# nirvanesque/headCT_foundation

Measured on AMD Instinct MI355X. Metric: CT-volumes/sec MAE pretrain step (96^3, ViT-B/16^3, mask 0.75), higher is better.
Workload: dtype bf16; 1 GPU; BASELINE config #2: MAE ViT-B/16^3, 96^3x1ch, mask 0.75, full train step (fwd+bwd+clip+AdamW+LR); per_gpu_batch=256, global_batch=256, parallelism=dp1, init=reference init, seed 42

## Files before the change

### headct_foundation_amd/_lib.py

```python
from __future__ import annotations

import ctypes as C
import os
from typing import Optional

HERE = os.path.dirname(os.path.abspath(__file__))
LIB_PATH = os.path.join(HERE, "libheadct_hip.so")

HCT_F32, HCT_BF16, HCT_F16 = 0, 1, 2
NORM_LAYERNORM, NORM_RMSNORM = 0, 1
HCT_ACT_NONE, HCT_ACT_GELU, HCT_ACT_DGELU, HCT_ACT_TANH, HCT_ACT_GELU_D, HCT_ACT_MULAUX = 0, 1, 2, 3, 4, 5
ACT_NONE, ACT_GELU, ACT_DGELU = 0, 1, 2

c_void_p, c_int, c_float, c_size_t, c_int64 = C.c_void_p, C.c_int, C.c_float, C.c_size_t, C.c_int64


class GemmArgs(C.Structure):
    _fields_ = [
        ("M", c_int), ("N", c_int), ("K", c_int),
        ("A", c_void_p), ("a_dtype", c_int), ("lda", c_int64), ("transA", c_int),
        ("B", c_void_p), ("b_dtype", c_int), ("ldb", c_int64), ("transB", c_int),
        ("C", c_void_p), ("c_dtype", c_int), ("ldc", c_int64),
        ("bias", c_void_p), ("residual", c_void_p), ("ldr", c_int64),
        ("act", c_int),
# ... 58 lines not shown
    "hct_rmsnorm_fwd": (c_int, [c_void_p, c_void_p, c_int, c_int, c_float, c_void_p, c_int, c_void_p, c_void_p]),
    "hct_rmsnorm_bwd_workspace_bytes": (c_size_t, [c_int, c_int]),
    "hct_rmsnorm_bwd": (c_int, [c_void_p, c_int, c_void_p, c_void_p, c_void_p, c_void_p, c_int, c_int, c_void_p, c_void_p, c_int, c_void_p,
                                c_void_p, c_void_p, c_size_t, c_void_p]),
    "hct_rmsnorm_bwd_mapped": (c_int, [c_void_p, c_int, c_void_p, c_void_p, c_void_p, c_void_p, c_void_p, c_int, c_int, c_void_p, c_void_p,
                                       c_int, c_void_p, c_void_p, c_void_p, c_size_t, c_void_p]),
    "hct_tail_rows": (c_int, [c_void_p, c_int, c_int, c_int, c_void_p, c_void_p, c_void_p]),
    "hct_gather_rows": (c_int, [c_void_p, c_void_p, c_int, c_int, c_void_p, c_void_p]),
    "hct_attention_fwd": (c_int, [c_void_p, c_int, c_int, c_int, c_int, c_int, c_void_p, c_void_p, c_void_p]),
    "hct_attention_bwd": (c_int, [c_void_p, c_void_p, c_void_p, c_void_p, c_int, c_int, c_int, c_int, c_int, c_void_p, c_void_p]),
    "hct_debug_force_simple_attention": (None, [c_int]),
    "hct_decoder_assemble_fwd": (c_int, [c_void_p, c_int, c_void_p, c_void_p, c_void_p, c_void_p, c_int, c_int, c_int, c_int, c_void_p, c_void_p]),
    "hct_decoder_assemble_bwd": (c_int, [c_void_p, c_void_p, c_void_p, c_int, c_int, c_int, c_int, c_void_p, c_int, c_void_p, c_void_p,
                                         c_void_p, c_size_t, c_void_p]),
    "hct_masked_mse": (c_int, [c_void_p, c_int, c_void_p, c_int, c_void_p, c_int, c_int, c_int, c_int, c_int, c_float, c_void_p, c_void_p, c_void_p, c_void_p, c_void_p]),
    "hct_unpatchify": (c_int, [c_void_p, c_int, c_int, c_int, c_int, c_int, c_int, c_void_p, c_void_p]),
    "hct_vit_assemble_fwd": (c_int, [c_void_p, c_int, c_void_p, c_void_p, c_void_p, c_int, c_int, c_int, c_int, c_void_p, c_void_p]),
    "hct_channel_norm": (c_int, [c_void_p, c_void_p, c_void_p, c_float, c_void_p, c_int, c_int64, c_int, c_void_p]),
    "hct_query_attention": (c_int, [c_void_p, c_int, c_void_p, c_int, c_int, c_int, c_int, c_int, c_float, c_void_p, c_void_p]),
    "hct_head_linear": (c_int, [c_void_p, c_int64, c_int, c_void_p, c_void_p, c_float, c_void_p, c_void_p, c_int, c_void_p, c_int, c_int,
                                c_int, c_void_p]),
    "hct_batchnorm_stats": (c_int, [c_void_p, c_int, c_int, c_float, c_void_p, c_void_p, c_void_p, c_void_p, c_void_p]),
    "hct_softmax_xent": (c_int, [c_void_p, c_void_p, c_int, c_int, c_void_p, c_void_p, c_void_p, c_void_p]),
    "hct_head_linear_wgrad": (c_int, [c_void_p, c_void_p, c_void_p, c_float, c_void_p, c_int, c_int, c_int, c_void_p, c_void_p, c_void_p]),
    "hct_bn_rows_workspace_bytes": (c_size_t, [c_int, c_int]),
    "hct_bn_stats_rows": (c_int, [c_void_p, c_int, c_int64, c_int, c_int, c_float, c_void_p, c_void_p, c_void_p, c_void_p, c_void_p,
                                  c_size_t, c_void_p]),
    "hct_bn_norm": (c_int, [c_void_p, c_int, c_int64, c_int64, c_int, c_void_p, c_void_p, c_float, c_void_p, c_int, c_void_p]),
    "hct_bn_bwd_input": (c_int, [c_void_p, c_int, c_int64, c_void_p, c_void_p, c_float, c_void_p, c_int64, c_void_p, c_void_p, c_int,
                                 c_int, c_int, c_int, c_void_p, c_int, c_int64, c_void_p, c_size_t, c_void_p]),
    "hct_head_linear_x": (c_int, [c_void_p, c_int, c_int64, c_int, c_void_p, c_void_p, c_float, c_void_p, c_void_p, c_void_p, c_int,
                                  c_int, c_int, c_void_p]),
    "hct_head_linear_bwd": (c_int, [c_void_p, c_int, c_int64, c_int, c_void_p, c_void_p, c_float, c_void_p, c_int, c_int, c_int,
                                    c_void_p, c_void_p, c_void_p]),
    "hct_query_attention_lse": (c_int, [c_void_p, c_int, c_void_p, c_int, c_int, c_int, c_int, c_int, c_float, c_void_p, c_void_p,
                                        c_void_p]),
    "hct_query_attention_bwd_workspace_bytes": (c_size_t, [c_int, c_int, c_int, c_int]),
    "hct_query_attention_bwd": (c_int, [c_void_p, c_int, c_void_p, c_int, c_int, c_int, c_int, c_int, c_float, c_void_p, c_void_p,
                                        c_void_p, c_void_p, c_void_p, c_void_p, c_size_t, c_void_p]),
    "hct_clip_total_norm": (c_int, [c_void_p, c_int64, c_void_p, c_int, c_float, c_void_p, c_void_p]),
    "hct_add_f32": (c_int, [c_void_p, c_void_p, c_int64, c_void_p]),
    "hct_dino_loss_workspace_bytes": (c_size_t, [c_int, c_int, c_int]),
    "hct_dino_loss": (c_int, [c_void_p, c_void_p, c_int, c_int, c_int, c_int, c_void_p, c_float, c_float, c_void_p, c_void_p, c_void_p, c_void_p,
                              c_void_p, c_size_t, c_void_p]),
    "hct_dino_center_update": (c_int, [c_void_p, c_void_p, c_int, C.c_double, C.c_double, c_void_p]),
    "hct_ema_update": (c_int, [c_void_p, c_void_p, c_int64, C.c_double, c_void_p]),
    "hct_l2norm_rows_fwd": (c_int, [c_void_p, c_int, c_int, c_void_p, c_int, c_void_p, c_void_p]),
    "hct_l2norm_rows_bwd": (c_int, [c_void_p, c_void_p, c_int, c_void_p, c_int, c_int, c_void_p, c_void_p]),
    "hct_weight_norm_fwd": (c_int, [c_void_p, c_void_p, c_int, c_int, c_void_p, c_int, c_void_p, c_void_p]),
    "hct_weight_norm_bwd": (c_int, [c_void_p, c_void_p, c_void_p, c_void_p, c_int, c_int, c_void_p, c_void_p, c_void_p]),
    "hct_bn_gelu_fwd": (c_int, [c_void_p, c_void_p, c_void_p, c_void_p, c_void_p, c_float, c_int, c_int, c_void_p, c_int, c_void_p, c_void_p, c_void_p]),
    "hct_bn_gelu_bwd_sums": (c_int, [c_void_p, c_int, c_void_p, c_void_p, c_int, c_int, c_void_p, c_void_p]),
    "hct_bn_gelu_bwd_apply": (c_int, [c_void_p, c_int, c_void_p, c_void_p, c_void_p, c_void_p, c_float, c_void_p, C.c_double, c_int, c_int, c_void_p, c_int,
                                      c_void_p]),
    "hct_hu_window": (c_int, [c_void_p, c_int, c_void_p, c_int, c_int, c_int64, c_int, c_void_p, c_void_p, c_void_p]),
    "hct_augment_volume": (c_int, [c_void_p, c_int, c_void_p, c_int, c_int, c_int, c_void_p, c_void_p, c_void_p]),
    "hct_gather_augment": (c_int, [c_void_p, c_void_p, c_void_p, c_int, c_int, c_int, c_int64, c_void_p, c_void_p, c_void_p]),
    "hct_gaussian_smooth3d": (c_int, [c_void_p, c_void_p, c_void_p, c_int, c_int, c_int, c_void_p, c_void_p, c_void_p]),
    "hct_crop_resize_area": (c_int, [c_void_p, c_int, c_int, c_int, c_int, c_void_p, c_int, c_int, c_void_p, c_void_p, c_void_p, c_void_p]),
    "hct_adjust_contrast_workspace_bytes": (c_size_t, [c_int, c_int64]),
    "hct_adjust_contrast": (c_int, [c_void_p, c_int, c_int64, c_void_p, c_void_p, c_void_p, c_size_t, c_void_p]),
    "hct_volume_to_ras": (c_int, [c_void_p, c_int, c_int, c_int, c_int, C.POINTER(c_int), C.POINTER(c_int), c_int, C.c_double, C.c_double,
                                  c_void_p, c_void_p]),
    "hct_bspline3_resample_workspace_bytes": (c_size_t, [c_int] * 6),
    "hct_bspline3_resample": (c_int, [c_void_p, c_int, c_int, c_int, c_void_p, c_int, c_int, c_int, c_void_p, c_void_p, c_void_p, c_size_t, c_void_p]),
    "hct_foreground_bbox_workspace_bytes": (c_size_t, [c_int] * 3),
    "hct_foreground_bbox": (c_int, [c_void_p, c_int, c_int, c_int, c_void_p, c_void_p, c_void_p, c_size_t, c_void_p]),
    "hct_crop_window_resize_area": (c_int, [c_void_p, c_int, c_int, c_int, c_void_p, c_int, c_void_p, c_void_p, c_void_p, c_int, c_int, c_int,
                                            c_void_p]),
    "hct_pos_embed_interp3d": (c_int, [c_void_p, c_int, c_void_p, c_int, c_int, c_int, c_void_p]),
    "hct_colsum_workspace_bytes": (c_size_t, [c_int, c_int]),
    "hct_colsum": (c_int, [c_void_p, c_int, c_int, c_int, c_int64, c_void_p, c_void_p, c_size_t, c_void_p]),
    "hct_cast": (c_int, [c_void_p, c_int, c_void_p, c_int, c_int64, c_void_p]),
    "hct_transpose_cast": (c_int, [c_void_p, c_int, c_void_p, c_int, c_int, c_int, c_void_p]),
    "hct_grad_norms_workspace_bytes": (c_size_t, [c_int64]),
    "hct_grad_norms": (c_int, [c_void_p, c_void_p, c_int, c_int64, c_float, c_int, c_void_p, c_void_p, c_void_p, c_size_t, c_void_p]),
    "hct_adamw_step": (c_int, [c_void_p, c_void_p, c_void_p, c_void_p, c_void_p, c_void_p, c_void_p, c_int, c_int64, c_float, c_float,
                               c_float, c_float, c_float, c_int, c_void_p, c_void_p]),
    "hct_lion_step": (c_int, [c_void_p] * 6 + [c_int, c_int64] + [C.c_double] * 4 + [c_void_p, c_void_p]),
    "hct_sgd_step": (c_int, [c_void_p] * 6 + [c_int, c_int64] + [C.c_double] * 2 + [c_void_p, c_void_p]),
    "hct_lamb_workspace_bytes": (c_size_t, [c_int64, c_int]),
    "hct_lamb_step": (c_int, [c_void_p] * 7 + [c_int, c_int64] + [C.c_double] * 5 + [c_void_p] * 4 + [c_size_t, c_void_p, c_void_p]),
    "hct_debug_set_gemm_variant": (None, [c_int]),
    "hct_gemm_nt_stream_k_bytes": (c_size_t, []),
    "hct_gemm_tn_group_workspace_bytes": (c_size_t, [c_int]),
    "hct_gemm_tn_group_prepare": (c_int, [c_void_p, c_int, c_void_p, c_size_t, c_void_p]),
    "hct_gemm_tn_group_run": (c_int, [c_void_p, c_int, c_void_p, c_size_t, c_void_p]),
    "hct_prof_enable": (None, [c_int]),
    "hct_prof_reset": (None, []),
    "hct_prof_read": (c_int, [c_int, C.POINTER(C.c_double), C.POINTER(c_int64), C.POINTER(C.c_double)]),
    "hct_prof_read_bytes": (c_int, [c_int, C.POINTER(C.c_double)]),
    "hct_prof_shapes": (c_int, [c_int, c_void_p, c_int]),
    "hct_mae_plan_create": (c_void_p, [C.POINTER(MaeConfig), c_int, c_int]),
    "hct_mae_plan_destroy": (None, [c_void_p]),
    "hct_mae_plan_num_params": (c_int, [c_void_p]),
    "hct_mae_plan_param_info": (c_int, [c_void_p, c_int, C.POINTER(ParamInfo)]),
    "hct_mae_plan_param_elems": (c_int64, [c_void_p]),
    "hct_mae_plan_bf16_t_elems": (c_int64, [c_void_p]),
    "hct_mae_plan_workspace_bytes": (c_size_t, [c_void_p]),
    "hct_mae_plan_len_keep": (c_int, [c_void_p]),
    "hct_mae_plan_set_tail": (c_int, [c_void_p, c_int]),
    "hct_mae_plan_set_dec0": (c_int, [c_void_p, c_int]),
    "hct_mae_backward_final_offset": (c_int64, [c_void_p]),
    "hct_mae_plan_set_wgrad_defer": (c_int, [c_void_p, c_int, c_int]),
    "hct_mae_plan_set_requires_grad": (c_int, [c_void_p, c_int, c_int]),
    "hct_lora_qv_fwd": (c_int, [c_void_p, c_void_p, c_void_p, c_void_p, c_void_p, c_int, c_int, c_int, c_int, c_int, c_int, c_void_p, c_void_p, c_void_p]),
    "hct_lora_qv_bwd_workspace_bytes": (c_size_t, [c_int, c_int, c_int, c_int]),
    "hct_lora_qv_bwd": (c_int, [c_void_p] * 11 + [c_int] * 6 + [c_void_p] * 6 + [c_size_t, c_void_p]),
    "hct_topk_dot_chunks": (c_int, [c_int, c_int64]),
    "hct_topk_dot_workspace": (c_size_t, [c_int, c_int64, c_int]),
    "hct_topk_dot": (c_int, [c_void_p, c_int, c_void_p, c_int64, c_int, c_int, c_void_p, c_int, c_void_p, c_void_p, c_void_p, c_size_t, c_void_p]),
    "hct_attention_row_probs": (c_int, [c_void_p, c_int, c_int, c_int, c_int, c_int, c_void_p, c_int, c_void_p, c_void_p]),
    "hct_mae_recon_accum": (c_int, [c_void_p, c_int, c_int, c_void_p, c_int, c_void_p, c_int, c_int, c_int, c_int, c_int, c_void_p, c_void_p, c_void_p,
                                    c_void_p]),
    "hct_mae_recon_finish": (c_int, [c_void_p, c_void_p, c_void_p, c_void_p, c_int, c_int, c_int, c_int, c_int, c_void_p, c_void_p, c_void_p, c_void_p]),
    "hct_mae_plan_bind": (c_int, [c_void_p, c_void_p, c_void_p, c_void_p, c_void_p, c_void_p, c_size_t]),
    "hct_mae_refresh_weights": (c_int, [c_void_p, c_int, c_void_p]),
    "hct_mae_forward": (c_int, [c_void_p, c_void_p, c_int, c_void_p, c_void_p, c_float, c_void_p]),
    "hct_mae_set_loss_grad": (c_int, [c_void_p, c_void_p]),
    "hct_mae_num_backward_stages": (c_int, [c_void_p]),
    "hct_mae_backward_stage_range": (c_int, [c_void_p, c_int, C.POINTER(c_int64), C.POINTER(c_int64)]),
    "hct_mae_backward_stage": (c_int, [c_void_p, c_int, c_void_p]),
    "hct_vit_forward": (c_int, [c_void_p, c_void_p, c_int, c_void_p]),
    "hct_vit_forward_parts": (c_int, [c_void_p, C.POINTER(c_void_p), c_int, c_int, c_void_p]),
    "hct_vit_backward_stage": (c_int, [c_void_p, c_int, c_void_p, c_void_p]),
    "hct_vit_assemble_bwd": (c_int, [c_void_p, c_int, c_int, c_int, c_int, c_void_p, c_int, c_void_p, c_void_p, c_void_p, c_void_p]),
    "hct_mae_plan_activation": (c_void_p, [c_void_p, C.c_char_p, C.POINTER(c_int64), C.POINTER(c_int64), C.POINTER(c_int)]),
}

_lib: Optional[C.CDLL] = None


class HctError(RuntimeError):
    pass


def exported_symbols():
    return sorted(_PROTOS)


def load() -> C.CDLL:
    global _lib
    if _lib is not None:
        return _lib
    if not os.path.exists(LIB_PATH):
        raise HctError(
            f"{LIB_PATH} not found: build it with `python -m headct_foundation_amd.build` "
            "(hipcc --offload-arch=gfx950).  There is no CPU fallback for the MAE hot path.")
    lib = C.CDLL(LIB_PATH)
    for name, (res, args) in _PROTOS.items():
        fn = getattr(lib, name)
        fn.restype = res
        fn.argtypes = args
    _lib = lib
    return lib


def check(rc: int, what: str = "") -> None:
    if rc != 0:
        msg = load().hct_last_error_string()
        raise HctError(f"{what} failed (rc={rc}): {msg.decode() if msg else ''}")


def ptr(t) -> Optional[int]:
    if t is None:
        return None
# ... 49 lines not shown
```

### headct_foundation_amd/csrc/common.h

```cpp
#pragma once
#include <hip/hip_runtime.h>
#include <stdint.h>
#include <stdio.h>
#include <string.h>

#include "../../include/headct_hip.h"

namespace hct {

typedef __bf16 bf16;
typedef _Float16 f16;
typedef __attribute__((ext_vector_type(4))) _Float16 f16x4;
typedef __attribute__((ext_vector_type(8))) __bf16 bf16x8;
typedef __attribute__((ext_vector_type(4))) __bf16 bf16x4;
typedef __attribute__((ext_vector_type(2))) __bf16 bf16x2;
typedef __attribute__((ext_vector_type(4))) short s16x4;
typedef __attribute__((ext_vector_type(4))) float f32x4;
typedef __attribute__((ext_vector_type(16))) float f32x16;

constexpr int kWave = 64;

void set_error(const char* fmt, ...);
int check_hip(hipError_t e, const char* what);
#define HCT_CHECK_LAUNCH(what)                         \
  do {                                                 \
    int _rc = ::hct::check_hip(hipGetLastError(), what); \
    if (_rc) return _rc;                               \
  } while (0)
#define HCT_REQUIRE(cond, ...)       \
  do {                               \
    if (!(cond)) {                   \
      ::hct::set_error(__VA_ARGS__); \
      return HCT_E_BADARG;           \
    }                                \
  } while (0)

int masked_mse_launch(const void* pred, int pred_dtype, const void* x, int x_dtype, const float* mask, int B, int C, int S, int P,
                      int norm_pix, float mask_sum, float* row_loss, float* loss, void* dpred, const float* dpred_scale,
                      float host_scale, hipStream_t s, const int32_t* masked_ids = nullptr, int K = 0);
int dec0_index(const int32_t* ids_restore, int B, int L, int K, int32_t* kept_rows, int32_t* cat_idx, hipStream_t s);
int dec0_table(const float* mask_token, const float* pos, int L, int D, float* out, hipStream_t s);
int dec0_aggregate(const void* g, int dtype, const int32_t* kept_rows, const int32_t* ids_restore, int B, int L, int K, int W, void* out, hipStream_t s);
int dec0_token_grads(const float* dh, const int32_t* ids_shuffle, const float* dcat, int B, int L, int K, int D, float* dmask, float* dcls,
                     void* workspace, size_t workspace_bytes, hipStream_t s);
bool tn_group_ok(const hct_gemm_args* a);
int lora_scatter(const void* T, int ldt, const void* Bq, const void* Bv, int B, int N, int H, int dh, int r, int dt, void* qkv, hipStream_t s);
int lora_gather(const void* dqkv, int B, int N, int H, int dh, int dt, void* dU, hipStream_t s);
int lora_dx_accum(const void* dT, int ldt, const void* Aq, const void* Av, bool transposed, int M, int D, int r, int dt, void* dx1, hipStream_t s);
int scale_unless_one(void* buf, int dtype, int64_t n, const float* scale, hipStream_t s);
int fold_rows(const float* partial, int nblk, int D, float* out, hipStream_t s);

struct FoldJob {
  const float* partial;
  int nblk, nq_stride, D, nq;
  float* out[3];
};
struct FoldSink {
  static constexpr int kMax = 8;
  FoldJob jobs[kMax];
  int n = 0;
};
extern thread_local FoldSink* g_fold_sink;
int fold_partials(const FoldJob& job, hipStream_t s);
int fold_flush(FoldSink& sink, hipStream_t s);

inline size_t dtype_size(int dt) { return dt == HCT_BF16 ? 2 : 4; }
inline size_t align_up(size_t v, size_t a) { return (v + a - 1) / a * a; }

__device__ __forceinline__ float to_f32(float v) { return v; }
__device__ __forceinline__ float to_f32(bf16 v) { return (float)v; }
template <typename T> __device__ __forceinline__ T from_f32(float v);
template <> __device__ __forceinline__ float from_f32<float>(float v) { return v; }
template <> __device__ __forceinline__ bf16 from_f32<bf16>(float v) { return (bf16)v; }

template <typename T> struct Vec4;
template <> struct Vec4<float> {
  static __device__ __forceinline__ f32x4 load(const float* p) { return *reinterpret_cast<const f32x4*>(p); }
  static __device__ __forceinline__ void store(float* p, f32x4 v) { *reinterpret_cast<f32x4*>(p) = v; }
  static __device__ __forceinline__ f32x4 load_nt(const float* p) { return __builtin_nontemporal_load(reinterpret_cast<const f32x4*>(p)); }
  static __device__ __forceinline__ void store_nt(float* p, f32x4 v) { __builtin_nontemporal_store(v, reinterpret_cast<f32x4*>(p)); }
};
template <> struct Vec4<bf16> {
  static __device__ __forceinline__ f32x4 load(const bf16* p) {
    bf16x4 v = *reinterpret_cast<const bf16x4*>(p);
    return f32x4{(float)v[0], (float)v[1], (float)v[2], (float)v[3]};
  }
  static __device__ __forceinline__ void store(bf16* p, f32x4 v) {
    bf16x4 o = {(bf16)v[0], (bf16)v[1], (bf16)v[2], (bf16)v[3]};
    *reinterpret_cast<bf16x4*>(p) = o;
  }
  static __device__ __forceinline__ f32x4 load_nt(const bf16* p) {
    bf16x4 v = __builtin_nontemporal_load(reinterpret_cast<const bf16x4*>(p));
    return f32x4{(float)v[0], (float)v[1], (float)v[2], (float)v[3]};
  }
  static __device__ __forceinline__ void store_nt(bf16* p, f32x4 v) {
    bf16x4 o = {(bf16)v[0], (bf16)v[1], (bf16)v[2], (bf16)v[3]};
    __builtin_nontemporal_store(o, reinterpret_cast<bf16x4*>(p));
  }
};

template <> struct Vec4<f16> {
  static __device__ __forceinline__ f32x4 load(const f16* p) {
    f16x4 v = *reinterpret_cast<const f16x4*>(p);
    return f32x4{(float)v[0], (float)v[1], (float)v[2], (float)v[3]};
  }
  static __device__ __forceinline__ void store(f16* p, f32x4 v) {
    f16x4 o = {(f16)v[0], (f16)v[1], (f16)v[2], (f16)v[3]};
    *reinterpret_cast<f16x4*>(p) = o;
  }
  static __device__ __forceinline__ f32x4 load_nt(const f16* p) {
    f16x4 v = __builtin_nontemporal_load(reinterpret_cast<const f16x4*>(p));
    return f32x4{(float)v[0], (float)v[1], (float)v[2], (float)v[3]};
  }
};
__device__ __forceinline__ float to_f32(f16 v) { return (float)v; }

__device__ __forceinline__ float wave_sum(float v) {
#pragma unroll
  for (int o = 32; o > 0; o >>= 1) v += __shfl_xor(v, o, 64);
  return v;
}
__device__ __forceinline__ float wave_max(float v) {
#pragma unroll
  for (int o = 32; o > 0; o >>= 1) v = fmaxf(v, __shfl_xor(v, o, 64));
  return v;
}

__device__ __forceinline__ float gelu_erf(float x) { return 0.5f * x * (1.0f + erff(x * 0.70710678118654752440f)); }
__device__ __forceinline__ float dgelu_erf(float x) {
  const float cdf = 0.5f * (1.0f + erff(x * 0.70710678118654752440f));
  const float pdf = 0.39894228040143267794f * __expf(-0.5f * x * x);
  return cdf + x * pdf;
}

__device__ __forceinline__ float gelu_cdf_poly(float x) {
  const float xc = __builtin_amdgcn_fmed3f(x, -4.0f, 4.0f);
  const float s = xc * xc;
  float p = fmaf(-1.4272797388414915e-09f, s, 1.1287725243391833e-07f);
  p = fmaf(p, s, -3.897907390637556e-06f);
  p = fmaf(p, s, 7.829771493561566e-05f);
  p = fmaf(p, s, -0.0010334221879020333f);
  p = fmaf(p, s, 0.009617664851248264f);
  p = fmaf(p, s, -0.06610910594463348f);
  p = fmaf(p, s, 0.398820698261261f);
  return fmaf(xc, p, 0.5f);
}
__device__ __forceinline__ float gelu_fast(float x) { return x * gelu_cdf_poly(x); }
// ... 51 lines not shown
```

### headct_foundation_amd/csrc/elementwise.hip

```cpp
#include "common.h"

#include <stdarg.h>
#include <algorithm>

namespace hct {

static thread_local char g_err[512] = "";
void set_error(const char* fmt, ...) {
  va_list ap;
  va_start(ap, fmt);
  vsnprintf(g_err, sizeof(g_err), fmt, ap);
  va_end(ap);
}
int check_hip(hipError_t e, const char* what) {
  if (e == hipSuccess) return 0;
  set_error("%s: %s", what, hipGetErrorString(e));
  return (int)e;
}

__global__ void mask_rank_kernel(const float* __restrict__ noise, int L, int K, int32_t* __restrict__ ids_restore,
                                 int32_t* __restrict__ ids_shuffle, float* __restrict__ mask) {
  extern __shared__ float s_noise[];
  const int b = blockIdx.x;
  const float* row = noise + (size_t)b * L;
  for (int i = threadIdx.x; i < L; i += blockDim.x) s_noise[i] = row[i];
  __syncthreads();
  for (int l = threadIdx.x; l < L; l += blockDim.x) {
    const float v = s_noise[l];
    int r = 0;
    for (int j = 0; j < L; ++j) {
      const float w = s_noise[j];
      r += (w < v) || (w == v && j < l);
    }
    ids_restore[(size_t)b * L + l] = r;
    ids_shuffle[(size_t)b * L + r] = l;
    mask[(size_t)b * L + l] = r < K ? 0.0f : 1.0f;
  }
}

template <typename TX, typename T>
__global__ void patch_gather_kernel(const TX* __restrict__ x, const int32_t* __restrict__ ids_shuffle, int C, int S,
                                    int P, int L, int K, T* __restrict__ rows) {
  const int r = blockIdx.x;
  const int b = r / K, j = r - b * K;
  const int g = S / P;
  const int l = ids_shuffle ? ids_shuffle[(size_t)b * L + j] : j;
  const int gh = l / (g * g), gw = (l / g) % g, gd = l % g;
  const int P4 = P >> 2;
  const int nvec = C * P * P * P4;
  T* out = rows + (size_t)r * (C * P * P * P);
  for (int v = threadIdx.x; v < nvec; v += blockDim.x) {
    int t = v;
    const int q = t % P4; t /= P4;
    const int pw = t % P; t /= P;
    const int ph = t % P; t /= P;
    const int c = t;
    const TX* src = x + ((((size_t)b * C + c) * S + (gh * P + ph)) * S + (gw * P + pw)) * S + gd * P + q * 4;
    Vec4<T>::store(out + (size_t)v * 4, Vec4<TX>::load(src));
  }
}

template <typename TX, typename T>
__global__ void __launch_bounds__(256) patch_gather_pencil_kernel(const TX* __restrict__ x, int C, int S, int P, T* __restrict__ rows) {
  extern __shared__ __attribute__((aligned(16))) unsigned char pg_smem[];
  T* lds = reinterpret_cast<T*>(pg_smem);
  const int g = S / P, P2 = P * P, P3 = P2 * P;
  int w = blockIdx.x;
  const int gw = w % g; w /= g;
  const int gh = w % g; w /= g;
  const int c = w % C;
  const int b = w / C;
  const TX* src = x + ((((size_t)b * C + c) * S + gh * P) * S + gw * P) * S;
  const int S4 = S >> 2;
  for (int v = threadIdx.x; v < P2 * S4; v += blockDim.x) {
    const int r = v / S4, e = (v - r * S4) * 4;
    const int ph = r / P, pw = r - ph * P;
    const f32x4 val = Vec4<TX>::load(src + ((size_t)ph * S + pw) * S + e);
    const int gd = e / P, pd = e - gd * P;
    Vec4<T>::store(lds + gd * P3 + r * P + pd, val);
  }
  __syncthreads();
  const int L = g * g * g;
  const size_t row0 = (size_t)b * L + ((size_t)gh * g + gw) * g;
  const int P34 = P3 >> 2;
  for (int v = threadIdx.x; v < g * P34; v += blockDim.x) {
    const int gd = v / P34, k = (v - gd * P34) * 4;
    Vec4<T>::store(rows + (row0 + gd) * ((size_t)C * P3) + (size_t)c * P3 + k, Vec4<T>::load(lds + gd * P3 + k));
  }
}

template <typename T>
__global__ void encoder_assemble_fwd_kernel(const T* __restrict__ tok, const float* __restrict__ cls,
                                            const float* __restrict__ pos, const int32_t* __restrict__ ids_shuffle,
                                            int L, int K, int D, float* __restrict__ h0) {
  const int r = blockIdx.x;
  const int b = r / (K + 1), t = r - b * (K + 1);
  float* out = h0 + (size_t)r * D;
  if (t == 0) {
    for (int d = threadIdx.x * 4; d < D; d += blockDim.x * 4) Vec4<float>::store(out + d, Vec4<float>::load(cls + d));
    return;
  }
  const int j = t - 1;
  const int l = ids_shuffle[(size_t)b * L + j];
  const T* src = tok + ((size_t)b * K + j) * D;
  for (int d = threadIdx.x * 4; d < D; d += blockDim.x * 4) {
    f32x4 v = Vec4<T>::load(src + d);
    if (pos) v += Vec4<float>::load(pos + (size_t)l * D + d);
    Vec4<float>::store(out + d, v);
  }
}

template <typename T>
__global__ void encoder_assemble_bwd_tok_kernel(const float* __restrict__ dh0, int K, int D, T* __restrict__ dtok) {
  const int r = blockIdx.x;
  const int b = r / K, j = r - b * K;
  const float* src = dh0 + ((size_t)b * (K + 1) + 1 + j) * D;
  T* out = dtok + (size_t)r * D;
  for (int d = threadIdx.x * 4; d < D; d += blockDim.x * 4) Vec4<T>::store(out + d, Vec4<float>::load(src + d));
}

__global__ void encoder_assemble_bwd_pos_kernel(const float* __restrict__ dh0, const int32_t* __restrict__ ids_restore,
                                                int B, int L, int K, int D, float* __restrict__ dpos) {
  const int l = blockIdx.x;
  for (int d = threadIdx.x * 4; d < D; d += blockDim.x * 4) {
    f32x4 acc = {0, 0, 0, 0};
    for (int b0 = 0; b0 < B; b0 += 8) {
      int r[8];
      f32x4 v[8];
#pragma unroll
      for (int u = 0; u < 8; ++u) r[u] = b0 + u < B ? ids_restore[(size_t)(b0 + u) * L + l] : K;
#pragma unroll
      for (int u = 0; u < 8; ++u)
        v[u] = r[u] < K ? Vec4<float>::load(dh0 + ((size_t)(b0 + u) * (K + 1) + 1 + r[u]) * D + d) : f32x4{0, 0, 0, 0};
#pragma unroll
      for (int u = 0; u < 8; ++u)
        if (r[u] < K) acc += v[u];
    }
    Vec4<float>::store(dpos + (size_t)l * D + d, acc);
  }
}

template <typename T>
__global__ void vit_assemble_bwd_tok_kernel(const float* __restrict__ dh0, int L, int R, int D, T* __restrict__ dtok) {
  const int r = blockIdx.x;
  const int b = r / L, l = r - b * L;
  const float* src = dh0 + ((size_t)b * (1 + R + L) + 1 + R + l) * D;
  T* out = dtok + (size_t)r * D;
  for (int d = threadIdx.x * 4; d < D; d += blockDim.x * 4) Vec4<T>::store(out + d, Vec4<float>::load(src + d));
}

__global__ void strided_rowsum_kernel(const float* __restrict__ src, int B, size_t stride, int D, float* __restrict__ out) {
  const int d = blockIdx.x * blockDim.x + threadIdx.x;
  if (d >= D) return;
  float acc = 0.f;
  for (int b0 = 0; b0 < B; b0 += 16) {
    float v[16];
#pragma unroll
    for (int u = 0; u < 16; ++u) v[u] = b0 + u < B ? src[(size_t)(b0 + u) * stride + d] : 0.f;
#pragma unroll
    for (int u = 0; u < 16; ++u)
      if (b0 + u < B) acc += v[u];
  }
  out[d] = acc;
}

template <typename T>
__global__ void __launch_bounds__(256) layernorm_fwd_kernel(const float* __restrict__ x, const float* __restrict__ gamma,
                                                            const float* __restrict__ beta, int rows, int D, float eps,
                                                            T* __restrict__ y, float* __restrict__ mean,
                                                            float* __restrict__ rstd) {
  const int lane = threadIdx.x & 63;
  const int row = blockIdx.x * (blockDim.x >> 6) + (threadIdx.x >> 6);
  if (row >= rows) return;
  const float* xr = x + (size_t)row * D;
  float s = 0.f;
  for (int d = lane * 4; d < D; d += 256) {
    f32x4 v = Vec4<float>::load(xr + d);
    s += (v[0] + v[1]) + (v[2] + v[3]);
  }
  const float mu = wave_sum(s) / (float)D;
  float q = 0.f;
  for (int d = lane * 4; d < D; d += 256) {
    f32x4 v = Vec4<float>::load(xr + d) - mu;
    q += (v[0] * v[0] + v[1] * v[1]) + (v[2] * v[2] + v[3] * v[3]);
  }
  const float rs = rsqrtf(wave_sum(q) / (float)D + eps);
  if (lane == 0) {
    mean[row] = mu;
    rstd[row] = rs;
  }
  T* yr = y + (size_t)row * D;
  for (int d = lane * 4; d < D; d += 256) {
    f32x4 v = (Vec4<float>::load(xr + d) - mu) * rs;
    v = v * Vec4<float>::load(gamma + d) + Vec4<float>::load(beta + d);
    Vec4<T>::store(yr + d, v);
  }
}

template <typename T, int NV>
__global__ void __launch_bounds__(256) layernorm_fwd_reg_kernel(const float* __restrict__ x, const float* __restrict__ gamma,
                                                                const float* __restrict__ beta, int rows, int D, float eps,
                                                                T* __restrict__ y, float* __restrict__ mean,
                                                                float* __restrict__ rstd) {
  const int lane = threadIdx.x & 63;
  const int wid = blockIdx.x * 4 + (threadIdx.x >> 6), nw = gridDim.x * 4;
  f32x4 g[NV], bt[NV];
#pragma unroll
  for (int i = 0; i < NV; ++i) {
    const int d = lane * 4 + 256 * i;
    g[i] = d < D ? Vec4<float>::load(gamma + d) : f32x4{0, 0, 0, 0};
    bt[i] = d < D ? Vec4<float>::load(beta + d) : f32x4{0, 0, 0, 0};
  }
  for (int row = wid; row < rows; row += nw) {
    const float* xr = x + (size_t)row * D;
    f32x4 v[NV];
    float s = 0.f;
#pragma unroll
    for (int i = 0; i < NV; ++i) {
      const int d = lane * 4 + 256 * i;
      if (d < D) {
        v[i] = Vec4<float>::load_nt(xr + d);
        s += (v[i][0] + v[i][1]) + (v[i][2] + v[i][3]);
      }
    }
    const float mu = wave_sum(s) / (float)D;
    float q = 0.f;
#pragma unroll
    for (int i = 0; i < NV; ++i) {
      const int d = lane * 4 + 256 * i;
      if (d < D) {
        const f32x4 c = v[i] - mu;
        q += (c[0] * c[0] + c[1] * c[1]) + (c[2] * c[2] + c[3] * c[3]);
      }
    }
    const float rs = rsqrtf(wave_sum(q) / (float)D + eps);
    if (lane == 0) {
      mean[row] = mu;
      rstd[row] = rs;
    }
    T* yr = y + (size_t)row * D;
#pragma unroll
    for (int i = 0; i < NV; ++i) {
      const int d = lane * 4 + 256 * i;
      if (d < D) {
        f32x4 o = (v[i] - mu) * rs;
        o = o * g[i] + bt[i];
        Vec4<T>::store(yr + d, o);
      }
    }
  }
}

constexpr int kLnBwdBlocks = 1024;


template <typename T, typename TS, int NV>
__global__ void __launch_bounds__(256) layernorm_bwd_kernel(const T* __restrict__ dy, const float* __restrict__ x,
                                                            const float* __restrict__ mean, const float* __restrict__ rstd,
                                                            const float* __restrict__ gamma, const float* dres,
                                                            const int32_t* __restrict__ dres_rows,
                                                            int rows, int D, float* dx, TS* __restrict__ shadow,
                                                            float* __restrict__ partial, int want_colsum) {
  __shared__ float s_red[4][3][NV * 256];
  const int lane = threadIdx.x & 63, wave = threadIdx.x >> 6;
  const int wid = blockIdx.x * 4 + wave, nw = gridDim.x * 4;
  f32x4 g[NV], pg[NV], pb[NV], pc[NV];
#pragma unroll
  for (int i = 0; i < NV; ++i) {
    const int d = lane * 4 + 256 * i;
    g[i] = d < D ? Vec4<float>::load(gamma + d) : f32x4{0, 0, 0, 0};
    pg[i] = pb[i] = pc[i] = f32x4{0, 0, 0, 0};
  }
  for (int row = wid; row < rows; row += nw) {
    const float mu = mean[row], rs = rstd[row];
    const int rrow = dres_rows ? dres_rows[row] : row;
    f32x4 dyv[NV], xh[NV];
    float s1 = 0.f, s2 = 0.f;
#pragma unroll
    for (int i = 0; i < NV; ++i) {
      const int d = lane * 4 + 256 * i;
      if (d < D) {
        dyv[i] = Vec4<T>::load_nt(dy + (size_t)row * D + d);
        xh[i] = (Vec4<float>::load_nt(x + (size_t)row * D + d) - mu) * rs;
      } else {
        dyv[i] = xh[i] = f32x4{0, 0, 0, 0};
      }
      const f32x4 a = dyv[i] * g[i];
      const f32x4 bq = a * xh[i];
      s1 += (a[0] + a[1]) + (a[2] + a[3]);
      s2 += (bq[0] + bq[1]) + (bq[2] + bq[3]);
      pg[i] += dyv[i] * xh[i];
      pb[i] += dyv[i];
    }
    s1 = wave_sum(s1) / (float)D;
    s2 = wave_sum(s2) / (float)D;
#pragma unroll
    for (int i = 0; i < NV; ++i) {
      const int d = lane * 4 + 256 * i;
      if (d < D) {
        f32x4 v = (dyv[i] * g[i] - s1 - xh[i] * s2) * rs;
        if (dres && rrow >= 0) v += Vec4<float>::load_nt(dres + (size_t)rrow * D + d);
        Vec4<float>::store(dx + (size_t)row * D + d, v);
        if (shadow) Vec4<TS>::store(shadow + (size_t)row * D + d, v);
        pc[i] += v;
      }
    }
  }
#pragma unroll
  for (int i = 0; i < NV; ++i) {
#pragma unroll
    for (int e = 0; e < 4; ++e) {
      s_red[wave][0][i * 256 + lane * 4 + e] = pg[i][e];
      s_red[wave][1][i * 256 + lane * 4 + e] = pb[i][e];
      s_red[wave][2][i * 256 + lane * 4 + e] = pc[i][e];
    }
  }
  __syncthreads();
  const int nq = want_colsum ? 3 : 2;
  for (int idx = threadIdx.x; idx < nq * NV * 256; idx += 256) {
    const int qn = idx / (NV * 256), c = idx - qn * (NV * 256);
    if (c < D) {
      const float v = (s_red[0][qn][c] + s_red[1][qn][c]) + (s_red[2][qn][c] + s_red[3][qn][c]);
      partial[((size_t)blockIdx.x * 3 + qn) * D + c] = v;
    }
  }
}

constexpr int kFoldThreads = 512;
__global__ void __launch_bounds__(512) fold_partials_kernel(const float* __restrict__ partial, int nblk, int nq_stride, int D,
                                                            float* o0, float* o1, float* o2) {
  __shared__ float s_red[16][32];
// ... 100 lines not shown
    float s2 = 0.f;
#pragma unroll
    for (int i = 0; i < NV; ++i) {
      const int d = lane * 4 + 256 * i;
      f32x4 dyv;
      if (d < D) {
        dyv = Vec4<T>::load_nt(dy + (size_t)row * D + d);
        xh[i] = Vec4<float>::load_nt(x + (size_t)row * D + d) * rs;
      } else {
        dyv = xh[i] = f32x4{0, 0, 0, 0};
      }
      a[i] = dyv * g[i];
      const f32x4 bq = a[i] * xh[i];
      s2 += (bq[0] + bq[1]) + (bq[2] + bq[3]);
      pg[i] += dyv * xh[i];
    }
    s2 = wave_sum(s2) / (float)D;
#pragma unroll
    for (int i = 0; i < NV; ++i) {
      const int d = lane * 4 + 256 * i;
      if (d < D) {
        f32x4 v = (a[i] - xh[i] * s2) * rs;
        if (dres && rrow >= 0) v += Vec4<float>::load_nt(dres + (size_t)rrow * D + d);
        Vec4<float>::store(dx + (size_t)row * D + d, v);
        if (shadow) Vec4<TS>::store(shadow + (size_t)row * D + d, v);
        pc[i] += v;
      }
    }
  }
#pragma unroll
  for (int i = 0; i < NV; ++i) {
#pragma unroll
    for (int e = 0; e < 4; ++e) {
      s_red[wave][0][i * 256 + lane * 4 + e] = pg[i][e];
      s_red[wave][1][i * 256 + lane * 4 + e] = pc[i][e];
    }
  }
  __syncthreads();
  const int nq = want_colsum ? 2 : 1;
  for (int idx = threadIdx.x; idx < nq * NV * 256; idx += 256) {
    const int qn = idx / (NV * 256), c = idx - qn * (NV * 256);
    if (c < D) {
      const float v = (s_red[0][qn][c] + s_red[1][qn][c]) + (s_red[2][qn][c] + s_red[3][qn][c]);
      partial[((size_t)blockIdx.x * 2 + qn) * D + c] = v;
    }
  }
}

template <typename T>
__global__ void decoder_assemble_fwd_kernel(const T* __restrict__ e, const float* __restrict__ mask_token,
                                            const float* __restrict__ dec_cls, const float* __restrict__ dec_pos,
                                            const int32_t* __restrict__ ids_restore, int L, int K, int D,
                                            float* __restrict__ y) {
  const int r = blockIdx.x;
  const int b = r / (L + 1), t = r - b * (L + 1);
  float* out = y + (size_t)r * D;
  if (t == 0) {
    const T* src = e + (size_t)b * (K + 1) * D;
    for (int d = threadIdx.x * 4; d < D; d += blockDim.x * 4)
      Vec4<float>::store(out + d, Vec4<T>::load(src + d) + Vec4<float>::load(dec_cls + d));
    return;
  }
  const int l = t - 1;
  const int rk = ids_restore[(size_t)b * L + l];
  const T* src = e + ((size_t)b * (K + 1) + 1 + rk) * D;
  for (int d = threadIdx.x * 4; d < D; d += blockDim.x * 4) {
    f32x4 v = rk < K ? Vec4<T>::load(src + d) : Vec4<float>::load(mask_token + d);
    Vec4<float>::store(out + d, v + Vec4<float>::load(dec_pos + (size_t)l * D + d));
  }
}

template <typename T>
__global__ void decoder_assemble_bwd_kernel(const float* __restrict__ dy, const int32_t* __restrict__ ids_shuffle, int L,
                                            int K, int D, T* __restrict__ de) {
  const int r = blockIdx.x;
  const int b = r / (K + 1), t = r - b * (K + 1);
  const int srow = t == 0 ? 0 : 1 + ids_shuffle[(size_t)b * L + (t - 1)];
  const float* src = dy + ((size_t)b * (L + 1) + srow) * D;
  T* out = de + (size_t)r * D;
  for (int d = threadIdx.x * 4; d < D; d += blockDim.x * 4) Vec4<T>::store(out + d, Vec4<float>::load(src + d));
}

constexpr int kAsmBlocks = 256;
__global__ void decoder_assemble_bwd_reduce_kernel(const float* __restrict__ dy, const int32_t* __restrict__ ids_shuffle,
                                                   int B, int L, int K, int D, float* __restrict__ partial) {
  for (int d = threadIdx.x * 4; d < D; d += blockDim.x * 4) {
    f32x4 am = {0, 0, 0, 0}, ac = {0, 0, 0, 0};
    for (int b = blockIdx.x; b < B; b += gridDim.x) {
      const float* base = dy + (size_t)b * (L + 1) * D;
      ac += Vec4<float>::load(base + d);
      for (int j0 = K; j0 < L; j0 += 8) {
        int l[8];
        f32x4 v[8];
#pragma unroll
        for (int u = 0; u < 8; ++u) l[u] = j0 + u < L ? ids_shuffle[(size_t)b * L + j0 + u] : 0;
#pragma unroll
        for (int u = 0; u < 8; ++u) v[u] = Vec4<float>::load(base + (size_t)(1 + l[u]) * D + d);
#pragma unroll
        for (int u = 0; u < 8; ++u)
          if (j0 + u < L) am += v[u];
      }
    }
    Vec4<float>::store(partial + ((size_t)blockIdx.x * 2 + 0) * D + d, am);
    Vec4<float>::store(partial + ((size_t)blockIdx.x * 2 + 1) * D + d, ac);
  }
}

__device__ __forceinline__ float block_sum_256(float v, float* s_tmp) {
  v = wave_sum(v);
  __syncthreads();
  if ((threadIdx.x & 63) == 0) s_tmp[threadIdx.x >> 6] = v;
  __syncthreads();
  return (s_tmp[0] + s_tmp[1]) + (s_tmp[2] + s_tmp[3]);
}

template <typename TX, typename T>
__global__ void __launch_bounds__(256) masked_mse_kernel(const T* __restrict__ pred, const TX* __restrict__ x,
                                                         const float* __restrict__ mask, int C, int S, int P, int L,
                                                         int norm_pix, float inv_masksum, float* __restrict__ row_loss,
                                                         T* __restrict__ dpred, const float* __restrict__ dscale, float hscale,
                                                         const int32_t* __restrict__ masked_ids, int K) {
  __shared__ float s_tmp[4];
  const int r = blockIdx.x;
  const int pd = P * P * P * C;
  const T* prow = pred + (size_t)r * pd;
  T* drow = dpred ? dpred + (size_t)r * pd : nullptr;
  int b, l;
  size_t lrow;
  if (masked_ids) {
    const int Lm = L - K;
    b = r / Lm;
    l = masked_ids[(size_t)b * L + K + (r - b * Lm)];
    lrow = r;
  } else {
    b = r / (L + 1);
    const int t = r - b * (L + 1);
    if (t == 0) {
      if (drow)
        for (int k = threadIdx.x * 4; k < pd; k += 1024) Vec4<T>::store(drow + k, f32x4{0, 0, 0, 0});
      return;
    }
    l = t - 1;
    lrow = (size_t)b * L + l;
    const float m = mask[lrow];
    if (m == 0.f) {
      if (threadIdx.x == 0 && row_loss) row_loss[lrow] = 0.f;
      if (drow)
        for (int k = threadIdx.x * 4; k < pd; k += 1024) Vec4<T>::store(drow + k, f32x4{0, 0, 0, 0});
      return;
    }
  }
  const int g = S / P;
  const int gh = l / (g * g), gw = (l / g) % g, gd = l % g;
  const TX* vol = x + (size_t)b * C * S * S * S;
  auto tgt_at = [&](int k) -> float {
    const int c = k % C;
    int u = k / C;
    const int pz = u % P; u /= P;
    const int pw = u % P; u /= P;
    const int ph = u;
    return to_f32(vol[(((size_t)c * S + (gh * P + ph)) * S + (gw * P + pw)) * S + gd * P + pz]);
  };
  float mu = 0.f, rsd = 1.f;
  if (norm_pix) {
    float s = 0.f;
    for (int k = threadIdx.x; k < pd; k += 256) s += tgt_at(k);
    mu = block_sum_256(s, s_tmp) / (float)pd;
    float q = 0.f;
    for (int k = threadIdx.x; k < pd; k += 256) {
      const float dlt = tgt_at(k) - mu;
      q += dlt * dlt;
    }
    const float var = block_sum_256(q, s_tmp) / (float)(pd - 1);
    rsd = 1.0f / sqrtf(var + 1.0e-6f);
  }
  const float gscale = 2.0f * inv_masksum / (float)pd * (dscale ? *dscale : 1.0f) * hscale;
  float sse = 0.f;
  if (C == 1) {
    for (int k = threadIdx.x * 4; k < pd; k += 1024) {
      int u = k;
      const int pz = u % P; u /= P;
      const int pw = u % P; u /= P;
      const int ph = u;
      const TX* tp = vol + ((size_t)(gh * P + ph) * S + (gw * P + pw)) * S + gd * P + pz;
      f32x4 tv = Vec4<TX>::load(tp);
      tv = (tv - mu) * rsd;
      const f32x4 df = Vec4<T>::load(prow + k) - tv;
      sse += (df[0] * df[0] + df[1] * df[1]) + (df[2] * df[2] + df[3] * df[3]);
      if (drow) Vec4<T>::store(drow + k, df * gscale);
    }
  } else {
    for (int k = threadIdx.x; k < pd; k += 256) {
      const float df = to_f32(prow[k]) - (tgt_at(k) - mu) * rsd;
      sse += df * df;
      if (drow) drow[k] = from_f32<T>(df * gscale);
    }
  }
  sse = block_sum_256(sse, s_tmp);
  if (threadIdx.x == 0 && row_loss) row_loss[lrow] = sse / (float)pd;
}

__global__ void __launch_bounds__(256) loss_fold_kernel(const float* __restrict__ row_loss, int n, float inv_masksum,
                                                        float* __restrict__ loss) {
  __shared__ float s_tmp[4];
  float s = 0.f;
  for (int i0 = threadIdx.x; i0 < n; i0 += 256 * 8) {
    float v[8];
#pragma unroll
    for (int u = 0; u < 8; ++u) v[u] = i0 + u * 256 < n ? row_loss[i0 + u * 256] : 0.f;
#pragma unroll
    for (int u = 0; u < 8; ++u)
      if (i0 + u * 256 < n) s += v[u];
  }
  s = block_sum_256(s, s_tmp);
  if (threadIdx.x == 0) *loss = s * inv_masksum;
}

template <typename T>
__global__ void unpatchify_kernel(const T* __restrict__ pred, int has_cls, int C, int S, int P, float* __restrict__ vol) {
  const int g = S / P, L = g * g * g;
  const int r = blockIdx.x;
  const int b = r / L, l = r - b * L;
  const int gh = l / (g * g), gw = (l / g) % g, gd = l % g;
  const int pd = P * P * P * C;
  const T* prow = pred + ((size_t)b * (L + has_cls) + has_cls + l) * pd;
  for (int k = threadIdx.x; k < pd; k += blockDim.x) {
    const int c = k % C;
    int u = k / C;
    const int pz = u % P; u /= P;
    const int pw = u % P; u /= P;
    const int ph = u;
    vol[((((size_t)b * C + c) * S + (gh * P + ph)) * S + (gw * P + pw)) * S + gd * P + pz] = to_f32(prow[k]);
  }
}

template <typename T>
__global__ void __launch_bounds__(256) colsum_partial_kernel(const T* __restrict__ x, int rows, int cols, int64_t ld,
                                                             int rows_per_chunk, float* __restrict__ partial) {
  __shared__ float s_red[4][256];
  const int lane = threadIdx.x & 63, wave = threadIdx.x >> 6;
  const int c0 = blockIdx.x * 256 + lane * 4;
  const int r0 = blockIdx.y * rows_per_chunk;
  const int r1 = min(rows, r0 + rows_per_chunk);
  f32x4 acc = {0, 0, 0, 0};
  if (c0 < cols)
    for (int r = r0 + wave; r < r1; r += 4 * 8) {
      f32x4 v[8];
#pragma unroll
      for (int u = 0; u < 8; ++u) v[u] = r + 4 * u < r1 ? Vec4<T>::load(x + (size_t)(r + 4 * u) * ld + c0) : f32x4{0, 0, 0, 0};
#pragma unroll
      for (int u = 0; u < 8; ++u)
        if (r + 4 * u < r1) acc += v[u];
    }
#pragma unroll
  for (int e = 0; e < 4; ++e) s_red[wave][lane * 4 + e] = acc[e];
  __syncthreads();
  const int c = blockIdx.x * 256 + threadIdx.x;
  if (c < cols)
    partial[(size_t)blockIdx.y * cols + c] =
        (s_red[0][threadIdx.x] + s_red[1][threadIdx.x]) + (s_red[2][threadIdx.x] + s_red[3][threadIdx.x]);
}

template <typename TI, typename TO>
__global__ void cast_kernel(const TI* __restrict__ src, TO* __restrict__ dst, int64_t n) {
  const int64_t stride = (int64_t)gridDim.x * blockDim.x * 4;
  for (int64_t i = ((int64_t)blockIdx.x * blockDim.x + threadIdx.x) * 4; i < n; i += stride) {
    if (i + 4 <= n) {
      Vec4<TO>::store(dst + i, Vec4<TI>::load(src + i));
    } else {
      for (int64_t k = i; k < n; ++k) dst[k] = from_f32<TO>(to_f32(src[k]));
    }
  }
}

template <typename TI, typename TO>
__global__ void __launch_bounds__(256) transpose_cast_kernel(const TI* __restrict__ src, TO* __restrict__ dst, int rows,
                                                             int cols) {
  __shared__ float tile[64][65];
  const int r0 = blockIdx.y * 64, c0 = blockIdx.x * 64;
  const int tx = threadIdx.x & 63, ty = threadIdx.x >> 6;
  for (int i = ty; i < 64; i += 4) {
    const int r = r0 + i, c = c0 + tx;
    tile[i][tx] = (r < rows && c < cols) ? to_f32(src[(size_t)r * cols + c]) : 0.f;
  }
// ... 256 lines not shown
    const float cs = fmaxf(0.f, ((float)o[a] + 0.5f) * scale - 0.5f);
    i0[a] = (int)cs;
    i1[a] = min(i0[a] + 1, gs - 1);
    w1[a] = cs - (float)i0[a];
  }
  f32x4 acc = {0, 0, 0, 0};
#pragma unroll
  for (int a = 0; a < 2; ++a)
#pragma unroll
    for (int b = 0; b < 2; ++b)
#pragma unroll
      for (int e = 0; e < 2; ++e) {
        const float w = (a ? w1[0] : 1.f - w1[0]) * (b ? w1[1] : 1.f - w1[1]) * (e ? w1[2] : 1.f - w1[2]);
        const int64_t row = extra + ((int64_t)(a ? i1[0] : i0[0]) * gs + (b ? i1[1] : i0[1])) * gs + (e ? i1[2] : i0[2]);
        acc += w * Vec4<float>::load(src + row * D + c);
      }
  Vec4<float>::store(dst + (int64_t)tok * D + c, acc);
}
}

template <typename T>
__global__ void __launch_bounds__(256) scale_unless_one_kernel(T* __restrict__ buf, int64_t n4, const float* __restrict__ scale) {
  const float sc = *scale;
  if (sc == 1.0f) return;
  for (int64_t i = (int64_t)blockIdx.x * 256 + threadIdx.x; i < n4; i += (int64_t)gridDim.x * 256)
    Vec4<T>::store(buf + i * 4, Vec4<T>::load(buf + i * 4) * sc);
}

namespace hct {
__global__ void __launch_bounds__(256) tail_rows_kernel(const int32_t* __restrict__ ids_restore, int B, int L, int K,
                                                        int32_t* __restrict__ tail_rows, int32_t* __restrict__ tail_inv) {
  const int r = blockIdx.x * 256 + threadIdx.x;
  if (r >= B * (L + 1)) return;
  const int b = r / (L + 1), t = r - b * (L + 1);
  int c = -1;
  if (t > 0) {
    const int rank = ids_restore[(size_t)b * L + (t - 1)];
    if (rank >= K) {
      c = b * (L - K) + (rank - K);
      tail_rows[c] = r;
    }
  }
  tail_inv[r] = c;
}

__global__ void __launch_bounds__(256) gather_rows16_kernel(const uint4* __restrict__ src, const int32_t* __restrict__ idx, int n_rows,
                                                            int chunks, uint4* __restrict__ dst) {
  const int64_t total = (int64_t)n_rows * chunks;
  for (int64_t i = (int64_t)blockIdx.x * 256 + threadIdx.x; i < total; i += (int64_t)gridDim.x * 256) {
    const int r = (int)(i / chunks), c = (int)(i - (int64_t)r * chunks);
    const int sr = idx[r];
    uint4 v = {0u, 0u, 0u, 0u};
    if (sr >= 0) v = src[(size_t)sr * chunks + c];
    dst[i] = v;
  }
}

__global__ void __launch_bounds__(256) dec0_index_kernel(const int32_t* __restrict__ ids_restore, int B, int L, int K,
                                                         int32_t* __restrict__ kept_rows, int32_t* __restrict__ cat_idx) {
  const int r = blockIdx.x * 256 + threadIdx.x;
  const int Nc = B * (K + 1);
  if (r < L) kept_rows[Nc + r] = -1;
  if (r >= B * (L + 1)) return;
  const int b = r / (L + 1), t = r - b * (L + 1);
  int c;
  if (t == 0) c = b * (K + 1);
  else {
    const int rank = ids_restore[(size_t)b * L + (t - 1)];
    c = rank < K ? b * (K + 1) + 1 + rank : Nc + (t - 1);
  }
  if (c < Nc) kept_rows[c] = r;
  cat_idx[r] = c;
}

__global__ void __launch_bounds__(256) dec0_table_kernel(const float* __restrict__ mask_token, const float* __restrict__ pos, int D,
                                                         float* __restrict__ out) {
  const int l = blockIdx.x;
  for (int d = threadIdx.x * 4; d < D; d += 1024)
    Vec4<float>::store(out + (size_t)l * D + d, Vec4<float>::load(mask_token + d) + Vec4<float>::load(pos + (size_t)l * D + d));
}

template <typename T>
__global__ void __launch_bounds__(256) dec0_table_sum_kernel(const T* __restrict__ g, const int32_t* __restrict__ ids_restore, int B, int L, int K,
                                                             int W, T* __restrict__ out) {
  __shared__ f32x4 s_part[4][64];
  const int l = blockIdx.x, q = threadIdx.x & 63, vg = threadIdx.x >> 6;
  const int col = blockIdx.y * 256 + q * 4;
  f32x4 acc = {0, 0, 0, 0};
  if (col < W) {
    for (int b0 = vg; b0 < B; b0 += 32) {
      int rk[8];
      f32x4 v[8];
#pragma unroll
      for (int u = 0; u < 8; ++u) rk[u] = b0 + 4 * u < B ? ids_restore[(size_t)(b0 + 4 * u) * L + l] : -1;
#pragma unroll
      for (int u = 0; u < 8; ++u)
        v[u] = rk[u] >= K ? Vec4<T>::load(g + ((size_t)(b0 + 4 * u) * (L + 1) + 1 + l) * W + col) : f32x4{0, 0, 0, 0};
#pragma unroll
      for (int u = 0; u < 8; ++u) acc += v[u];
    }
  }
  s_part[vg][q] = acc;
  __syncthreads();
  if (vg == 0 && col < W) Vec4<T>::store(out + (size_t)l * W + col, (s_part[0][q] + s_part[1][q]) + (s_part[2][q] + s_part[3][q]));
}

__global__ void __launch_bounds__(512) dec0_token_grads_kernel(const float* __restrict__ partial, int nblk, const float* __restrict__ dcat,
                                                               int B, int L, int K, int D, float* __restrict__ dmask, float* __restrict__ dcls) {
  __shared__ float s_m[16][32], s_c[16][32];
  const int c = threadIdx.x & 31, rg = threadIdx.x >> 5;
  const int d = blockIdx.x * 32 + c;
  const size_t Nc = (size_t)B * (K + 1);
  auto sum_rows = [&](const float* base, int n, size_t stride) {
    float acc = 0.f;
    for (int r0 = rg; r0 < n; r0 += 16 * 8) {
      float v[8];
#pragma unroll
      for (int u = 0; u < 8; ++u) v[u] = r0 + 16 * u < n ? base[(size_t)(r0 + 16 * u) * stride + d] : 0.f;
#pragma unroll
      for (int u = 0; u < 8; ++u) acc += v[u];
    }
    return acc;
  };
  float m = 0.f, cl = 0.f;
  if (d < D) {
    m = sum_rows(partial, nblk, (size_t)2 * D) + sum_rows(dcat + Nc * D, L, D);
    cl = sum_rows(dcat, B, (size_t)(K + 1) * D);
  }
  s_m[rg][c] = m;
  s_c[rg][c] = cl;
  __syncthreads();
  if (rg == 0 && d < D) {
    float a = 0.f, bsum = 0.f;
#pragma unroll
    for (int i = 0; i < 16; ++i) { a += s_m[i][c]; bsum += s_c[i][c]; }
    dmask[d] = a;
    dcls[d] = bsum;
  }
}

int scale_unless_one(void* buf, int dtype, int64_t n, const float* scale, hipStream_t s) {
  HCT_REQUIRE(n % 4 == 0 && scale, "scale_unless_one: n %% 4 != 0 or null scale");
  const int blocks = (int)std::min<int64_t>(2048, (n / 4 + 255) / 256);
  if (blocks == 0) return 0;
  HCT_DISPATCH_DTYPE(dtype, T, hipLaunchKernelGGL(scale_unless_one_kernel<T>, dim3(blocks), dim3(256), 0, s, (T*)buf, n / 4, scale));
  HCT_CHECK_LAUNCH("scale_unless_one");
  return 0;
}

int masked_mse_launch(const void* pred, int pred_dtype, const void* x, int x_dtype, const float* mask, int B, int C, int S, int P,
                      int norm_pix, float mask_sum, float* row_loss, float* loss, void* dpred, const float* dpred_scale,
                      float host_scale, hipStream_t s, const int32_t* masked_ids, int K) {
  HCT_REQUIRE(P % 4 == 0 && S % P == 0 && mask_sum > 0.f, "hct_masked_mse: bad geometry S=%d P=%d mask_sum=%f", S, P, mask_sum);
  HCT_REQUIRE(x_dtype == HCT_F32 || x_dtype == HCT_F16, "hct_masked_mse: volumes are fp32 or fp16");
  const int g = S / P, L = g * g * g;
  const int pd = P * P * P * C;
  HCT_REQUIRE(pd % 4 == 0, "hct_masked_mse: patch dim %% 4 != 0");
  const float inv = 1.0f / mask_sum;
  HCT_REQUIRE(!masked_ids || (K >= 0 && K < L), "hct_masked_mse: compact form needs 0 <= K < L");
  const int nrows = masked_ids ? B * (L - K) : B * (L + 1);
  if (x_dtype == HCT_F16) {
    HCT_DISPATCH_DTYPE(pred_dtype, T,
                       hipLaunchKernelGGL((masked_mse_kernel<f16, T>), dim3(nrows), dim3(256), 0, s, (const T*)pred, (const f16*)x, mask,
                                          C, S, P, L, norm_pix, inv, loss ? row_loss : nullptr, (T*)dpred, dpred_scale, host_scale, masked_ids, K));
  } else
  HCT_DISPATCH_DTYPE(pred_dtype, T,
                     hipLaunchKernelGGL((masked_mse_kernel<float, T>), dim3(nrows), dim3(256), 0, s, (const T*)pred, (const float*)x, mask,
                                        C, S, P, L, norm_pix, inv, loss ? row_loss : nullptr, (T*)dpred, dpred_scale, host_scale, masked_ids, K));
  if (loss) hipLaunchKernelGGL(loss_fold_kernel, dim3(1), dim3(256), 0, s, row_loss, masked_ids ? B * (L - K) : B * L, inv, loss);
  HCT_CHECK_LAUNCH("hct_masked_mse");
  return 0;
}

int dec0_index(const int32_t* ids_restore, int B, int L, int K, int32_t* kept_rows, int32_t* cat_idx, hipStream_t s) {
  const int n = std::max(B * (L + 1), L);
  hipLaunchKernelGGL(dec0_index_kernel, dim3((n + 255) / 256), dim3(256), 0, s, ids_restore, B, L, K, kept_rows, cat_idx);
  HCT_CHECK_LAUNCH("dec0_index");
  return 0;
}
int dec0_table(const float* mask_token, const float* pos, int L, int D, float* out, hipStream_t s) {
  hipLaunchKernelGGL(dec0_table_kernel, dim3(L), dim3(256), 0, s, mask_token, pos, D, out);
  HCT_CHECK_LAUNCH("dec0_table");
  return 0;
}
int dec0_aggregate(const void* g, int dtype, const int32_t* kept_rows, const int32_t* ids_restore, int B, int L, int K, int W, void* out, hipStream_t s) {
  HCT_REQUIRE(W % 4 == 0 && (W * dtype_size(dtype)) % 16 == 0, "dec0_aggregate: row width must be a multiple of 16 bytes");
  const int Nc = B * (K + 1);
  if (int rc = hct_gather_rows(g, kept_rows, Nc, (int)(W * dtype_size(dtype)), out, s)) return rc;
  const dim3 grid(L, (W + 255) / 256);
  HCT_DISPATCH_DTYPE(dtype, T, hipLaunchKernelGGL(dec0_table_sum_kernel<T>, grid, dim3(256), 0, s, (const T*)g, ids_restore, B, L, K, W, (T*)out + (size_t)Nc * W));
  HCT_CHECK_LAUNCH("dec0_aggregate");
  return 0;
}
int dec0_token_grads(const float* dh, const int32_t* ids_shuffle, const float* dcat, int B, int L, int K, int D, float* dmask, float* dcls,
                     void* workspace, size_t workspace_bytes, hipStream_t s) {
  if (workspace_bytes < hct_assemble_bwd_workspace_bytes(D)) {
    set_error("dec0_token_grads: workspace too small");
    return HCT_E_WORKSPACE;
  }
  const int threads = D / 4 >= 256 ? 256 : (D / 4 > 64 ? 128 : 64);
  const int nblk = std::min(B, kAsmBlocks);
  float* partial = (float*)workspace;
  hipLaunchKernelGGL(decoder_assemble_bwd_reduce_kernel, dim3(nblk), dim3(threads), 0, s, dh, ids_shuffle, B, L, K, D, partial);
  hipLaunchKernelGGL(dec0_token_grads_kernel, dim3((D + 31) / 32), dim3(512), 0, s, partial, nblk, dcat, B, L, K, D, dmask, dcls);
  HCT_CHECK_LAUNCH("dec0_token_grads");
  return 0;
}
}

extern "C" {

const char* hct_last_error_string(void) { return g_err; }
int hct_version(void) { return 100; }
int hct_has_mfma_kernels(void) { return 1; }

int hct_mask_rank(const float* noise, int B, int L, int K, int32_t* ids_restore, int32_t* ids_shuffle, float* mask,
                  void* stream) {
  HCT_REQUIRE(B > 0 && L > 0 && K >= 0 && K <= L && L <= 12288, "hct_mask_rank: bad shape B=%d L=%d K=%d", B, L, K);
  hipLaunchKernelGGL(mask_rank_kernel, dim3(B), dim3(256), L * sizeof(float), (hipStream_t)stream, noise, L, K,
                     ids_restore, ids_shuffle, mask);
  HCT_CHECK_LAUNCH("hct_mask_rank");
  return 0;
}

int hct_patch_gather(const void* x, int x_dtype, const int32_t* ids_shuffle, int B, int C, int S, int P, int L, int K, void* rows,
                     int rows_dtype, void* stream) {
  HCT_REQUIRE(P % 4 == 0 && S % P == 0 && (S / P) * (S / P) * (S / P) == L, "hct_patch_gather: bad geometry S=%d P=%d L=%d", S, P, L);
  HCT_REQUIRE(x_dtype == HCT_F32 || x_dtype == HCT_F16, "hct_patch_gather: volumes are fp32 or fp16");
  if (B * K == 0) return 0;
  const size_t pencil_lds = (size_t)P * P * S * dtype_size(rows_dtype);
  if (!ids_shuffle && K == L && S % 4 == 0 && pencil_lds <= 64 * 1024) {
    const int g = S / P;
    if (x_dtype == HCT_F16) {
      HCT_DISPATCH_DTYPE(rows_dtype, T,
                         hipLaunchKernelGGL((patch_gather_pencil_kernel<f16, T>), dim3(B * C * g * g), dim3(256), pencil_lds, (hipStream_t)stream,
                                            (const f16*)x, C, S, P, (T*)rows));
    } else {
      HCT_DISPATCH_DTYPE(rows_dtype, T,
                         hipLaunchKernelGGL((patch_gather_pencil_kernel<float, T>), dim3(B * C * g * g), dim3(256), pencil_lds, (hipStream_t)stream,
                                            (const float*)x, C, S, P, (T*)rows));
    }
    HCT_CHECK_LAUNCH("hct_patch_gather(pencil)");
    return 0;
  }
  if (x_dtype == HCT_F16) {
    HCT_DISPATCH_DTYPE(rows_dtype, T,
                       hipLaunchKernelGGL((patch_gather_kernel<f16, T>), dim3(B * K), dim3(256), 0, (hipStream_t)stream, (const f16*)x,
                                          ids_shuffle, C, S, P, L, K, (T*)rows));
  } else
  HCT_DISPATCH_DTYPE(rows_dtype, T,
                     hipLaunchKernelGGL((patch_gather_kernel<float, T>), dim3(B * K), dim3(256), 0, (hipStream_t)stream, (const float*)x,
                                        ids_shuffle, C, S, P, L, K, (T*)rows));
  HCT_CHECK_LAUNCH("hct_patch_gather");
  return 0;
}

int hct_encoder_assemble_fwd(const void* tok, int tok_dtype, const float* cls, const float* pos,
                             const int32_t* ids_shuffle, int B, int L, int K, int D, float* h0, void* stream) {
  HCT_REQUIRE(D % 4 == 0, "hct_encoder_assemble_fwd: D %% 4 != 0 (%d)", D);
  const int threads = D / 4 >= 256 ? 256 : (D / 4 > 64 ? 128 : 64);
  HCT_DISPATCH_DTYPE(tok_dtype, T,
                     hipLaunchKernelGGL(encoder_assemble_fwd_kernel<T>, dim3(B * (K + 1)), dim3(threads), 0,
                                        (hipStream_t)stream, (const T*)tok, cls, pos, ids_shuffle, L, K, D, h0));
  HCT_CHECK_LAUNCH("hct_encoder_assemble_fwd");
  return 0;
}

size_t hct_assemble_bwd_workspace_bytes(int D) { return (size_t)kAsmBlocks * 2 * D * sizeof(float); }

int hct_encoder_assemble_bwd(const float* dh0, const int32_t* ids_restore, int B, int L, int K, int D, void* dtok,
                             int dtok_dtype, float* dcls, float* dpos, void* workspace, size_t workspace_bytes,
                             void* stream) {
  (void)workspace; (void)workspace_bytes;
  HCT_REQUIRE(D % 4 == 0, "hct_encoder_assemble_bwd: D %% 4 != 0 (%d)", D);
  const int threads = D / 4 >= 256 ? 256 : (D / 4 > 64 ? 128 : 64);
  hipStream_t s = (hipStream_t)stream;
  if (dtok && B * K > 0)
    HCT_DISPATCH_DTYPE(dtok_dtype, T,
                       hipLaunchKernelGGL(encoder_assemble_bwd_tok_kernel<T>, dim3(B * K), dim3(threads), 0, s, dh0, K, D,
                                          (T*)dtok));
  if (dcls) hipLaunchKernelGGL(strided_rowsum_kernel, dim3((D + 255) / 256), dim3(256), 0, s, dh0, B, (size_t)(K + 1) * D, D, dcls);
  if (dpos) hipLaunchKernelGGL(encoder_assemble_bwd_pos_kernel, dim3(L), dim3(threads), 0, s, dh0, ids_restore, B, L, K, D, dpos);
  HCT_CHECK_LAUNCH("hct_encoder_assemble_bwd");
  return 0;
}

int hct_vit_assemble_bwd(const float* dh0, int B, int L, int R, int D, void* dtok, int dtok_dtype, float* dcls, float* dreg, float* dpos,
                         void* stream) {
  HCT_REQUIRE(dh0 && B > 0 && L > 0 && R >= 0 && D > 0 && D % 4 == 0, "hct_vit_assemble_bwd: bad arguments");
  hipStream_t s = (hipStream_t)stream;
  const size_t stride = (size_t)(1 + R + L) * D;
  if (dtok) {
    HCT_DISPATCH_DTYPE(dtok_dtype, T, hipLaunchKernelGGL(hct::vit_assemble_bwd_tok_kernel<T>, dim3(B * L), dim3(D / 4 >= 256 ? 256 : 64), 0, s, dh0, L,
                                                        R, D, (T*)dtok));
  }
  if (dcls) hipLaunchKernelGGL(strided_rowsum_kernel, dim3((D + 255) / 256), dim3(256), 0, s, dh0, B, stride, D, dcls);
  if (dreg && R > 0) hipLaunchKernelGGL(strided_rowsum_kernel, dim3((R * D + 255) / 256), dim3(256), 0, s, dh0 + D, B, stride, R * D, dreg);
  if (dpos) hipLaunchKernelGGL(strided_rowsum_kernel, dim3((L * D + 255) / 256), dim3(256), 0, s, dh0 + (size_t)(1 + R) * D, B, stride, L * D, dpos);
  HCT_CHECK_LAUNCH("hct_vit_assemble_bwd");
  return 0;
}

int hct_layernorm_fwd(const float* x, const float* gamma, const float* beta, int rows, int D, float eps, void* y,
                      int y_dtype, float* mean, float* rstd, void* stream) {
  HCT_REQUIRE(D % 4 == 0 && rows >= 0, "hct_layernorm_fwd: bad shape rows=%d D=%d", rows, D);
  if (rows == 0) return 0;
  const int nblk = min((rows + 3) / 4, 2048);
#define HCT_LN_FWD(NV_)                                                                                                 \
  HCT_DISPATCH_DTYPE(y_dtype, T,                                                                                       \
                     hipLaunchKernelGGL((layernorm_fwd_reg_kernel<T, NV_>), dim3(nblk), dim3(256), 0, (hipStream_t)stream, x, \
                                        gamma, beta, rows, D, eps, (T*)y, mean, rstd))
  if (D <= 256) HCT_LN_FWD(1);
  else if (D <= 512) HCT_LN_FWD(2);
  else if (D <= 768) HCT_LN_FWD(3);
  else if (D <= 1024) HCT_LN_FWD(4);
  else
    HCT_DISPATCH_DTYPE(y_dtype, T,
                       hipLaunchKernelGGL(layernorm_fwd_kernel<T>, dim3((rows + 3) / 4), dim3(256), 0, (hipStream_t)stream,
                                          x, gamma, beta, rows, D, eps, (T*)y, mean, rstd));
#undef HCT_LN_FWD
  HCT_CHECK_LAUNCH("hct_layernorm_fwd");
  return 0;
}

size_t hct_layernorm_bwd_workspace_bytes(int rows, int D) {
  (void)rows;
  return (size_t)kLnBwdBlocks * 3 * D * sizeof(float);
}

int hct_layernorm_bwd(const void* dy, int dy_dtype, const float* x, const float* mean, const float* rstd,
                      const float* gamma, const float* dres, int rows, int D, float* dx, void* dx_shadow,
                      int shadow_dtype, float* dgamma, float* dbeta, float* dcolsum, void* workspace,
                      size_t workspace_bytes, void* stream) {
  return hct_layernorm_bwd_mapped(dy, dy_dtype, x, mean, rstd, gamma, dres, nullptr, rows, D, dx, dx_shadow, shadow_dtype, dgamma, dbeta,
                                  dcolsum, workspace, workspace_bytes, stream);
}

int hct_layernorm_bwd_mapped(const void* dy, int dy_dtype, const float* x, const float* mean, const float* rstd,
                             const float* gamma, const float* dres, const int32_t* dres_rows, int rows, int D, float* dx,
                             void* dx_shadow, int shadow_dtype, float* dgamma, float* dbeta, float* dcolsum, void* workspace,
                             size_t workspace_bytes, void* stream) {
  HCT_REQUIRE(D % 4 == 0 && rows > 0, "hct_layernorm_bwd: bad shape rows=%d D=%d", rows, D);
  HCT_REQUIRE(!dres_rows || (dres && (const void*)dres != (const void*)dx), "hct_layernorm_bwd_mapped: a mapped residual gradient cannot alias dx");
  if (workspace_bytes < hct_layernorm_bwd_workspace_bytes(rows, D)) {
    set_error("hct_layernorm_bwd: workspace too small");
    return HCT_E_WORKSPACE;
  }
  hipStream_t s = (hipStream_t)stream;
  const int nblk = min(kLnBwdBlocks, (rows + 3) / 4);
  float* partial = (float*)workspace;
  int rc = 0;
  if (dy_dtype == HCT_BF16) {
    if (dx_shadow && shadow_dtype == HCT_F32) rc = launch_ln_bwd<bf16, float>(dy, x, mean, rstd, gamma, dres, dres_rows, rows, D, dx, dx_shadow, partial, dcolsum != nullptr, nblk, s);
    else rc = launch_ln_bwd<bf16, bf16>(dy, x, mean, rstd, gamma, dres, dres_rows, rows, D, dx, dx_shadow, partial, dcolsum != nullptr, nblk, s);
  } else {
    if (dx_shadow && shadow_dtype == HCT_BF16) rc = launch_ln_bwd<float, bf16>(dy, x, mean, rstd, gamma, dres, dres_rows, rows, D, dx, dx_shadow, partial, dcolsum != nullptr, nblk, s);
    else rc = launch_ln_bwd<float, float>(dy, x, mean, rstd, gamma, dres, dres_rows, rows, D, dx, dx_shadow, partial, dcolsum != nullptr, nblk, s);
  }
  if (rc) return rc;
  HCT_CHECK_LAUNCH("hct_layernorm_bwd");
  return fold_partials(FoldJob{partial, nblk, 3, D, dcolsum ? 3 : 2, {dgamma, dbeta, dcolsum}}, s);
}

int hct_rmsnorm_fwd(const float* x, const float* gamma, int rows, int D, float eps, void* y, int y_dtype, float* rstd,
                    void* stream) {
  HCT_REQUIRE(D % 4 == 0 && rows >= 0, "hct_rmsnorm_fwd: bad shape rows=%d D=%d", rows, D);
  if (rows == 0) return 0;
  const int nblk = min((rows + 3) / 4, 2048);
#define HCT_RMS_FWD(NV_)                                                                                                     \
  HCT_DISPATCH_DTYPE(y_dtype, T,                                                                                             \
                     hipLaunchKernelGGL((rmsnorm_fwd_reg_kernel<T, NV_>), dim3(nblk), dim3(256), 0, (hipStream_t)stream, x, gamma, \
                                        rows, D, eps, (T*)y, rstd))
  if (D <= 256) HCT_RMS_FWD(1);
  else if (D <= 512) HCT_RMS_FWD(2);
  else if (D <= 768) HCT_RMS_FWD(3);
  else if (D <= 1024) HCT_RMS_FWD(4);
  else
    HCT_DISPATCH_DTYPE(y_dtype, T,
                       hipLaunchKernelGGL(rmsnorm_fwd_kernel<T>, dim3((rows + 3) / 4), dim3(256), 0, (hipStream_t)stream, x, gamma,
                                          rows, D, eps, (T*)y, rstd));
#undef HCT_RMS_FWD
  HCT_CHECK_LAUNCH("hct_rmsnorm_fwd");
  return 0;
}

size_t hct_rmsnorm_bwd_workspace_bytes(int rows, int D) { return hct_layernorm_bwd_workspace_bytes(rows, D); }

int hct_rmsnorm_bwd(const void* dy, int dy_dtype, const float* x, const float* rstd, const float* gamma, const float* dres, int rows,
                    int D, float* dx, void* dx_shadow, int shadow_dtype, float* dgamma, float* dcolsum, void* workspace,
                    size_t workspace_bytes, void* stream) {
  return hct_rmsnorm_bwd_mapped(dy, dy_dtype, x, rstd, gamma, dres, nullptr, rows, D, dx, dx_shadow, shadow_dtype, dgamma, dcolsum,
                                workspace, workspace_bytes, stream);
}

int hct_rmsnorm_bwd_mapped(const void* dy, int dy_dtype, const float* x, const float* rstd, const float* gamma, const float* dres,
                           const int32_t* dres_rows, int rows, int D, float* dx, void* dx_shadow, int shadow_dtype, float* dgamma,
                           float* dcolsum, void* workspace, size_t workspace_bytes, void* stream) {
  HCT_REQUIRE(D % 4 == 0 && rows > 0, "hct_rmsnorm_bwd: bad shape rows=%d D=%d", rows, D);
  HCT_REQUIRE(!dres_rows || (dres && (const void*)dres != (const void*)dx), "hct_rmsnorm_bwd_mapped: a mapped residual gradient cannot alias dx");
  if (workspace_bytes < hct_rmsnorm_bwd_workspace_bytes(rows, D)) {
    set_error("hct_rmsnorm_bwd: workspace too small");
    return HCT_E_WORKSPACE;
  }
  hipStream_t s = (hipStream_t)stream;
  const int nblk = min(kLnBwdBlocks, (rows + 3) / 4);
  float* partial = (float*)workspace;
  const int wc = dcolsum != nullptr;
  int rc = 0;
  if (dy_dtype == HCT_BF16) {
    if (dx_shadow && shadow_dtype == HCT_F32) rc = launch_rms_bwd<bf16, float>(dy, x, rstd, gamma, dres, dres_rows, rows, D, dx, dx_shadow, partial, wc, nblk, s);
    else rc = launch_rms_bwd<bf16, bf16>(dy, x, rstd, gamma, dres, dres_rows, rows, D, dx, dx_shadow, partial, wc, nblk, s);
  } else {
    if (dx_shadow && shadow_dtype == HCT_BF16) rc = launch_rms_bwd<float, bf16>(dy, x, rstd, gamma, dres, dres_rows, rows, D, dx, dx_shadow, partial, wc, nblk, s);
    else rc = launch_rms_bwd<float, float>(dy, x, rstd, gamma, dres, dres_rows, rows, D, dx, dx_shadow, partial, wc, nblk, s);
  }
  if (rc) return rc;
  HCT_CHECK_LAUNCH("hct_rmsnorm_bwd");
  return fold_partials(FoldJob{partial, nblk, 2, D, wc ? 2 : 1, {dgamma, dcolsum, nullptr}}, s);
}

int hct_decoder_assemble_fwd(const void* e, int e_dtype, const float* mask_token, const float* dec_cls,
                             const float* dec_pos, const int32_t* ids_restore, int B, int L, int K, int D, float* y,
                             void* stream) {
  HCT_REQUIRE(D % 4 == 0, "hct_decoder_assemble_fwd: D %% 4 != 0 (%d)", D);
  const int threads = D / 4 >= 256 ? 256 : (D / 4 > 64 ? 128 : 64);
  HCT_DISPATCH_DTYPE(e_dtype, T,
                     hipLaunchKernelGGL(decoder_assemble_fwd_kernel<T>, dim3(B * (L + 1)), dim3(threads), 0,
                                        (hipStream_t)stream, (const T*)e, mask_token, dec_cls, dec_pos, ids_restore, L, K,
                                        D, y));
  HCT_CHECK_LAUNCH("hct_decoder_assemble_fwd");
  return 0;
}

int hct_decoder_assemble_bwd(const float* dy, const int32_t* ids_restore, const int32_t* ids_shuffle, int B, int L,
                             int K, int D, void* de, int de_dtype, float* dmask_token, float* ddec_cls,
                             void* workspace, size_t workspace_bytes, void* stream) {
  (void)ids_restore;
  HCT_REQUIRE(D % 4 == 0, "hct_decoder_assemble_bwd: D %% 4 != 0 (%d)", D);
  if (workspace_bytes < hct_assemble_bwd_workspace_bytes(D)) {
    set_error("hct_decoder_assemble_bwd: workspace too small");
    return HCT_E_WORKSPACE;
  }
  hipStream_t s = (hipStream_t)stream;
  const int threads = D / 4 >= 256 ? 256 : (D / 4 > 64 ? 128 : 64);
  HCT_DISPATCH_DTYPE(de_dtype, T,
                     hipLaunchKernelGGL(decoder_assemble_bwd_kernel<T>, dim3(B * (K + 1)), dim3(threads), 0, s, dy,
                                        ids_shuffle, L, K, D, (T*)de));
  const int nblk = min(B, kAsmBlocks);
  float* partial = (float*)workspace;
  hipLaunchKernelGGL(decoder_assemble_bwd_reduce_kernel, dim3(nblk), dim3(threads), 0, s, dy, ids_shuffle, B, L, K, D, partial);
  hipLaunchKernelGGL(fold_partials_kernel, dim3((D + 31) / 32, 2), dim3(kFoldThreads), 0, s, partial, nblk, 2, D, dmask_token,
                     ddec_cls, (float*)nullptr);
  HCT_CHECK_LAUNCH("hct_decoder_assemble_bwd");
  return 0;
}

int hct_masked_mse(const void* pred, int pred_dtype, const void* x, int x_dtype, const float* mask, int B, int C, int S, int P,
                   int norm_pix, float mask_sum, float* row_loss, float* loss, void* dpred, const float* dpred_scale,
                   void* stream) {
  return masked_mse_launch(pred, pred_dtype, x, x_dtype, mask, B, C, S, P, norm_pix, mask_sum, row_loss, loss, dpred, dpred_scale, 1.0f,
                           (hipStream_t)stream, nullptr, 0);
}

int hct_tail_rows(const int32_t* ids_restore, int B, int L, int K, int32_t* tail_rows, int32_t* tail_inv, void* stream) {
  HCT_REQUIRE(ids_restore && tail_rows && tail_inv && B > 0 && L > 0 && K >= 0 && K < L, "hct_tail_rows: bad arguments");
  const int n = B * (L + 1);
  hipLaunchKernelGGL(hct::tail_rows_kernel, dim3((n + 255) / 256), dim3(256), 0, (hipStream_t)stream, ids_restore, B, L, K, tail_rows, tail_inv);
  HCT_CHECK_LAUNCH("hct_tail_rows");
  return 0;
}

int hct_gather_rows(const void* src, const int32_t* idx, int n_rows, int row_bytes, void* dst, void* stream) {
  HCT_REQUIRE(src && idx && dst && n_rows >= 0 && row_bytes > 0 && row_bytes % 16 == 0 && ((uintptr_t)src % 16) == 0 && ((uintptr_t)dst % 16) == 0,
              "hct_gather_rows: bad arguments (rows of a multiple of 16 bytes, 16-byte aligned)");
  if (n_rows == 0) return 0;
  const int64_t total = (int64_t)n_rows * (row_bytes / 16);
  const int blocks = (int)std::min<int64_t>(8192, (total + 255) / 256);
  hipLaunchKernelGGL(hct::gather_rows16_kernel, dim3(blocks), dim3(256), 0, (hipStream_t)stream, (const uint4*)src, idx, n_rows, row_bytes / 16, (uint4*)dst);
  HCT_CHECK_LAUNCH("hct_gather_rows");
  return 0;
}

int hct_unpatchify(const void* pred, int pred_dtype, int has_cls_row, int B, int C, int S, int P, float* vol,
                   void* stream) {
  HCT_REQUIRE(S % P == 0, "hct_unpatchify: bad geometry");
  const int g = S / P, L = g * g * g;
  HCT_DISPATCH_DTYPE(pred_dtype, T,
                     hipLaunchKernelGGL(unpatchify_kernel<T>, dim3(B * L), dim3(256), 0, (hipStream_t)stream,
                                        (const T*)pred, has_cls_row ? 1 : 0, C, S, P, vol));
  HCT_CHECK_LAUNCH("hct_unpatchify");
  return 0;
}

static int colsum_chunks(int rows, int cols) {
  const int colblk = (cols + 255) / 256;
  int chunks = (1024 + colblk - 1) / colblk;
  if (chunks > (rows + 15) / 16) chunks = (rows + 15) / 16;
  return chunks < 1 ? 1 : chunks;
}
size_t hct_colsum_workspace_bytes(int rows, int cols) { return (size_t)colsum_chunks(rows, cols) * cols * sizeof(float); }

int hct_colsum(const void* x, int dtype, int rows, int cols, int64_t ld, float* out, void* workspace,
               size_t workspace_bytes, void* stream) {
  HCT_REQUIRE(cols % 4 == 0 && ld % 4 == 0 && rows > 0, "hct_colsum: cols/ld must be multiples of 4");
  if (workspace_bytes < hct_colsum_workspace_bytes(rows, cols)) {
    set_error("hct_colsum: workspace too small");
    return HCT_E_WORKSPACE;
  }
  hipStream_t s = (hipStream_t)stream;
  const int chunks = colsum_chunks(rows, cols);
  const int rpc = (rows + chunks - 1) / chunks;
  float* partial = (float*)workspace;
  HCT_DISPATCH_DTYPE(dtype, T,
                     hipLaunchKernelGGL(colsum_partial_kernel<T>, dim3((cols + 255) / 256, chunks), dim3(256), 0, s,
                                        (const T*)x, rows, cols, ld, rpc, partial));
  hipLaunchKernelGGL(fold_partials_kernel, dim3((cols + 31) / 32, 1), dim3(kFoldThreads), 0, s, partial, chunks, 1, cols, out,
                     (float*)nullptr, (float*)nullptr);
  HCT_CHECK_LAUNCH("hct_colsum");
  return 0;
}

int hct_cast(const void* src, int src_dtype, void* dst, int dst_dtype, int64_t n, void* stream) {
  if (n <= 0) return 0;
  hipStream_t s = (hipStream_t)stream;
  const int blocks = (int)std::min<int64_t>(2048, (n + 1023) / 1024);
  if (src_dtype == HCT_F32 && dst_dtype == HCT_BF16)
    hipLaunchKernelGGL((cast_kernel<float, bf16>), dim3(blocks), dim3(256), 0, s, (const float*)src, (bf16*)dst, n);
  else if (src_dtype == HCT_BF16 && dst_dtype == HCT_F32)
    hipLaunchKernelGGL((cast_kernel<bf16, float>), dim3(blocks), dim3(256), 0, s, (const bf16*)src, (float*)dst, n);
  else if (src_dtype == HCT_F32)
    hipLaunchKernelGGL((cast_kernel<float, float>), dim3(blocks), dim3(256), 0, s, (const float*)src, (float*)dst, n);
  else
    hipLaunchKernelGGL((cast_kernel<bf16, bf16>), dim3(blocks), dim3(256), 0, s, (const bf16*)src, (bf16*)dst, n);
// ... 88 lines not shown
```

### headct_foundation_amd/csrc/gemm.hip

```cpp
#include "common.h"
#include "prof.h"

#include <cstdlib>
#include <cstring>
#include <vector>

namespace hct {

static int g_nt_variant = 0;
static int g_mt3 = 1;
static int g_sk_drop = 0;

struct Epilogue {
  const float* bias;
  const float* residual;
  int64_t ldr;
  int act;
  void* aux; int aux_dtype; int64_t ldaux;
  void* C; int c_dtype; int64_t ldc;
  void* C2; int c2_dtype; int64_t ldc2;
  float alpha;
  float* colsum_partial;
  int aux_deriv;
};
// ... 1530 lines not shown
      __builtin_amdgcn_raw_ptr_buffer_load_lds(rb, (lds_void*)(base + 16384 + c * 1024), 16, ob, 0, 0, 0);
    }
  };

  const int wr = wave >> 1, wc = wave & 1;
  const int g = lane >> 4, q = (lane & 15) >> 2, pp = lane & 3;
  const int f = q | ((g & 1) << 2);
  const int row_base = (8 * g + q) * 256 + pp * 8;
  f32x4 acc[4][4];
#pragma unroll
  for (int i = 0; i < 4; ++i)
#pragma unroll
    for (int j = 0; j < 4; ++j) acc[i][j] = f32x4{0, 0, 0, 0};

  auto frag = [&](const unsigned char* tile, int nb, int ks) -> bf16x8 {
    const unsigned char* p = tile + row_base + ks * (32 * 256) + ((nb ^ f) << 5);
    s16x4 lo = __builtin_amdgcn_ds_read_tr16_b64_v4i16((__attribute__((address_space(3))) s16x4*)(p));
    s16x4 hi = __builtin_amdgcn_ds_read_tr16_b64_v4i16((__attribute__((address_space(3))) s16x4*)(p + 4 * 256));
    typedef __attribute__((ext_vector_type(8))) short s16x8;
    s16x8 v = {lo[0], lo[1], lo[2], lo[3], hi[0], hi[1], hi[2], hi[3]};
    return __builtin_bit_cast(bf16x8, v);
  };

  const int nsteps = (rend - rbeg + 63) >> 6;
  if (nsteps > 0) {
    stage(0, 0);
    __syncthreads();
    for (int t = 0; t < nsteps; ++t) {
      const int buf = t & 1;
      if (t + 1 < nsteps) stage(buf ^ 1, (t + 1) << 6);
      const unsigned char* ta = smem + buf * 32768;
      const unsigned char* tb = ta + 16384;
#pragma unroll
      for (int ks = 0; ks < 2; ++ks) {
        bf16x8 af[4], bfr[4];
#pragma unroll
        for (int i = 0; i < 4; ++i) af[i] = frag(ta, wr * 4 + i, ks);
#pragma unroll
        for (int j = 0; j < 4; ++j) bfr[j] = frag(tb, wc * 4 + j, ks);
#pragma unroll
        for (int i = 0; i < 4; ++i)
#pragma unroll
          for (int j = 0; j < 4; ++j) acc[i][j] = __builtin_amdgcn_mfma_f32_16x16x32_bf16(bfr[j], af[i], acc[i][j], 0, 0, 0);
      }
      __syncthreads();
    }
  }
  Epilogue eo = e;
  if (slab) {
    eo.bias = nullptr; eo.residual = nullptr; eo.act = HCT_ACT_NONE; eo.aux = nullptr; eo.C2 = nullptr; eo.alpha = 1.0f;
    eo.C = slab + (int64_t)blockIdx.y * M * N; eo.c_dtype = HCT_F32; eo.ldc = N;
  }
#pragma unroll
  for (int i = 0; i < 4; ++i)
    epilogue_tile16x64(eo, smem + wave * kStageBytes, lane, m0 + wr * 64 + i * 16, n0 + wc * 64, M, N, acc[i]);
}

__global__ void __launch_bounds__(256) gemm_fold_kernel(const float* __restrict__ slab, int splits, int M, int N, Epilogue e) {
  const int64_t total4 = (int64_t)M * N / 4;
  for (int64_t i = (int64_t)blockIdx.x * blockDim.x + threadIdx.x; i < total4; i += (int64_t)gridDim.x * blockDim.x) {
    const int64_t idx = i * 4;
    f32x4 s = Vec4<float>::load_nt(slab + idx);
    for (int z = 1; z < splits; ++z) s += Vec4<float>::load_nt(slab + (int64_t)z * M * N + idx);
    const int m = (int)(idx / N), n = (int)(idx - (int64_t)m * N);
    epilogue4(e, m, n, s);
  }
}

static int g_cu_reserve = 0;

static int num_cus_total() {
  static int n = 0;
  if (n == 0) {
    int dev = 0;
    hipDeviceProp_t prop;
    if (hipGetDevice(&dev) == hipSuccess && hipGetDeviceProperties(&prop, dev) == hipSuccess) n = prop.multiProcessorCount;
    if (n <= 0) n = 256;
  }
  return n;
}

static int num_cus() { return std::max(8, num_cus_total() - g_cu_reserve); }

static bool aligned_to(const void* p, size_t a) { return p == nullptr || ((uintptr_t)p % a) == 0; }

static Epilogue make_epilogue(const hct_gemm_args* a) {
  Epilogue e;
  e.bias = a->bias; e.residual = a->residual; e.ldr = a->ldr;
  e.aux_deriv = a->act == HCT_ACT_GELU_D || a->act == HCT_ACT_MULAUX;
  e.act = a->act == HCT_ACT_GELU_D ? HCT_ACT_GELU : a->act == HCT_ACT_MULAUX ? HCT_ACT_DGELU : a->act;
  e.aux = a->aux; e.aux_dtype = a->aux_dtype; e.ldaux = a->ldaux;
  e.C = a->C; e.c_dtype = a->c_dtype; e.ldc = a->ldc;
  e.C2 = a->C2; e.c2_dtype = a->c2_dtype; e.ldc2 = a->ldc2;
  e.alpha = a->alpha;
  e.colsum_partial = nullptr;
  return e;
}

static bool epilogue_vec_ok(const hct_gemm_args* a) {
  auto ok = [](const void* p, int dt, int64_t ld) { return p == nullptr || (ld % 4 == 0 && aligned_to(p, dt == HCT_BF16 ? 8 : 16)); };
  return a->N % 4 == 0 && ok(a->C, a->c_dtype, a->ldc) && ok(a->C2, a->c2_dtype, a->ldc2) && ok(a->aux, a->aux_dtype, a->ldaux) &&
         ok(a->residual, HCT_F32, a->ldr) && aligned_to(a->bias, 16);
}

enum Path { PATH_GENERIC = 0, PATH_NT = 1, PATH_TN = 2 };

static Path choose_path(const hct_gemm_args* a) {
  if (a->force_generic || a->a_dtype != HCT_BF16 || a->b_dtype != HCT_BF16) return PATH_GENERIC;
  if (!epilogue_vec_ok(a)) return PATH_GENERIC;
  if (!aligned_to(a->A, 16) || !aligned_to(a->B, 16) || a->lda % 8 || a->ldb % 8) return PATH_GENERIC;
  if (a->transA == 0 && a->transB == 1 && a->K % 64 == 0 && a->N % 16 == 0 && a->lda * 2 * 128 < (1ll << 31) && a->ldb * 2 * 128 < (1ll << 31))
    return PATH_NT;
  if (a->transA == 1 && a->transB == 0 && a->M % 16 == 0 && a->N % 16 == 0 && a->act == HCT_ACT_NONE && !a->bias && !a->residual &&
      (int64_t)a->K * a->lda * 2 < (1ll << 40))
    return PATH_TN;
  return PATH_GENERIC;
}

static bool tn256_ok(const hct_gemm_args* a) {
  return g_nt_variant != 128 && a->c_dtype == HCT_F32 && !a->C2 && a->ldc % 4 == 0 && a->ldc * 256 < (1ll << 28) &&
         a->lda * 2 * 64 < (1ll << 31) && a->ldb * 2 * 64 < (1ll << 31);
}

static void tn256_split(const hct_gemm_args* a, int& splits, int& r_chunk) {
  const int tiles = ((a->M + 255) / 256) * ((a->N + 255) / 256);
  int s = std::max(1, num_cus() / tiles);
  int per = (a->K + s - 1) / s;
  per = std::max(128, (per + 63) / 64 * 64);
  while ((int64_t)per * std::max(a->lda, a->ldb) * 2 >= (1ll << 31)) per = std::max(128, per / 2 / 64 * 64);
  r_chunk = per;
  splits = (a->K + per - 1) / per;
}

static int epilogue_mode(const hct_gemm_args* a) {
  if (a->C2) return EPI_GENERIC;
  const bool small = a->ldc * 256 < (1ll << 28) && a->ldr * 256 < (1ll << 28) && a->ldaux * 256 < (1ll << 28);
  if (!small) return EPI_GENERIC;
  auto wide_ok = [](const void* p, int64_t ld) { return p == nullptr || (ld % 8 == 0 && aligned_to(p, 16)); };
  if (a->c_dtype == HCT_BF16 && !(a->N % 8 == 0 && wide_ok(a->C, a->ldc) && wide_ok(a->aux, a->ldaux))) return EPI_GENERIC;
  if (a->act == HCT_ACT_NONE && !a->residual && a->c_dtype == HCT_BF16) return EPI_PLAIN_BF16;
  if (a->act == HCT_ACT_NONE && a->residual && a->c_dtype == HCT_F32) return EPI_RES_F32;
  const bool is_gelu = a->act == HCT_ACT_GELU || a->act == HCT_ACT_GELU_D, is_dgelu = a->act == HCT_ACT_DGELU || a->act == HCT_ACT_MULAUX;
  if (is_gelu && !a->residual && a->c_dtype == HCT_BF16 && a->aux && a->aux_dtype == HCT_BF16) return EPI_GELU_BF16;
  if (is_dgelu && !a->residual && a->c_dtype == HCT_BF16 && a->aux_dtype == HCT_BF16) return EPI_DGELU_BF16;
  return EPI_GENERIC;
}

static int g_sk_min_k = 512;
static int g_sk_gain_pairs = 20;
static bool nt_stream_k(const hct_gemm_args* a, int tiles256, int& sk_tiles, int& sk_wgs) {
  sk_tiles = sk_wgs = 0;
  const int G = num_cus(), P = a->K / 64;
  if (G > kSkMaxWgs || a->K < g_sk_min_k || P < 8 || P > 1023) return false;
  const int rem = tiles256 % G;
  if (rem == 0 || (int64_t)(G - rem) * P < (int64_t)g_sk_gain_pairs * G) return false;
  const int gx = G / 8, nxmax = (rem + 7) / 8;
  if (G % 8 || (int64_t)nxmax * P > (int64_t)gx * (P - 1)) return false;
  sk_tiles = rem;
  sk_wgs = (int)std::min<int64_t>(gx, std::max<int64_t>(1, (int64_t)((rem + 7) / 8) * P / 4));
  return true;
}

static void tn_split(const hct_gemm_args* a, int& splits, int& r_chunk) {
  const int tiles = ((a->M + 127) / 128) * ((a->N + 127) / 128);
  const int steps = (a->K + 63) / 64;
  int s = (1024 + tiles - 1) / tiles;
// ... 400 lines not shown
```

### headct_foundation_amd/csrc/mae_plan.hip

```cpp
#include <cstdlib>
#include "common.h"

#include <algorithm>
#include <map>
#include <string>
#include <vector>

using namespace hct;

namespace {

constexpr int64_t kUnitElems = 1024;

struct BlockP {
  int ln1_w, ln1_b, qkv_w, qkv_b, proj_w, proj_b, ln2_w, ln2_b, fc1_w, fc1_b, fc2_w, fc2_b;
  int lq_b = -1, lq_a = -1, lv_b = -1, lv_a = -1;
};
struct BlockA {
  size_t x1, mean1, rstd1, qkv, o, lse, h_mid, x2, mean2, rstd2, u, g;
  size_t lora_t = 0;
};
struct Act { size_t off; int64_t rows, cols; int dtype; };
struct BlockG { size_t out, big, mid, qkv, lora_du = 0, lora_dt = 0; };
constexpr int kWgSlots = 8;
// ... 39 lines not shown
  int wg_blocks = 0;
  int wg_blocks_pending = 0, wg_slot = 0;
  std::vector<BlockG> genc, gdec;
  size_t a_de = 0, a_dtok = 0;
  std::vector<hct_gemm_args> wg_pending;
  std::vector<hct_gemm_args> wg_prepared[kWgSlots];
  size_t s_wg[kWgSlots] = {0}, s_wg_bytes = 0;
  int64_t final_off = 0;
  float* params_f32 = nullptr;
  float* grads = nullptr;
  bf16* params_bf16 = nullptr;
  bf16* params_bf16_t = nullptr;
  unsigned char* ws = nullptr;
  bool fwd_done = false;
  bool nt_ws_armed = false;
  bool dpred_done = false;
  const float* dloss = nullptr;

  size_t esz() const { return dtype_size(dt); }
  template <typename T> T* W(size_t off) const { return reinterpret_cast<T*>(ws + off); }
  const float* pf(int i) const { return i < 0 ? nullptr : params_f32 + params[i].offset; }
  float* gf(int i) const { return i < 0 ? nullptr : grads + params[i].offset; }
  const void* wop(int i) const { return dt == HCT_BF16 ? (const void*)(params_bf16 + params[i].offset) : (const void*)(params_f32 + params[i].offset); }
  const void* wop_t(int i) const { return (const void*)(params_bf16_t + params[i].bf16_t_offset); }
  int tr(int i) const { return i >= 0 && params[i].requires_grad ? i : -1; }
};

namespace {

int add_param(hct_mae_plan* p, const std::string& name, std::vector<int64_t> shape, bool rg, bool matrix, bool needs_t) {
  hct_param_info pi;
  memset(&pi, 0, sizeof(pi));
  snprintf(pi.name, sizeof(pi.name), "%s", name.c_str());
  pi.ndim = (int)shape.size();
  int64_t n = 1;
  for (size_t i = 0; i < shape.size(); ++i) { pi.shape[i] = shape[i]; n *= shape[i]; }
  pi.numel = n;
  pi.offset = p->param_elems;
  pi.requires_grad = rg ? 1 : 0;
  pi.is_matrix = matrix ? 1 : 0;
  pi.bf16_t_offset = -1;
  if (needs_t) {
    pi.bf16_t_offset = p->bf16t_elems;
    p->bf16t_elems += (n + 63) / 64 * 64;
  }
  p->param_elems += (n + kUnitElems - 1) / kUnitElems * kUnitElems;
  p->params.push_back(pi);
  p->pindex[name] = (int)p->params.size() - 1;
  return (int)p->params.size() - 1;
}

BlockP add_block(hct_mae_plan* p, const std::string& pre, int d, int m, bool use_bias) {
  BlockP b;
  b.ln1_w = add_param(p, pre + ".att_norm.weight", {d}, true, false, false);
  b.ln1_b = p->norm_kind == 1 ? -1 : add_param(p, pre + ".att_norm.bias", {d}, true, false, false);
  b.qkv_w = add_param(p, pre + ".attn.qkv.weight", {3 * d, d}, true, true, true);
  b.qkv_b = use_bias ? add_param(p, pre + ".attn.qkv.bias", {3 * d}, true, false, false) : -1;
  b.proj_w = add_param(p, pre + ".attn.proj.weight", {d, d}, true, true, true);
  b.proj_b = add_param(p, pre + ".attn.proj.bias", {d}, true, false, false);
  if (p->lora > 0) {
    const int r = p->lora;
    b.lq_b = add_param(p, pre + ".attn.lora_q.lora_matrix_B", {d, r}, true, true, true);
    b.lv_b = add_param(p, pre + ".attn.lora_v.lora_matrix_B", {d, r}, true, true, true);
    b.lq_a = add_param(p, pre + ".attn.lora_q.lora_matrix_A", {r, d}, true, true, true);
    b.lv_a = add_param(p, pre + ".attn.lora_v.lora_matrix_A", {r, d}, true, true, true);
  }
  b.ln2_w = add_param(p, pre + ".ffn_norm.weight", {d}, true, false, false);
  b.ln2_b = p->norm_kind == 1 ? -1 : add_param(p, pre + ".ffn_norm.bias", {d}, true, false, false);
  b.fc1_w = add_param(p, pre + ".mlp.linear1.weight", {m, d}, true, true, true);
  b.fc1_b = add_param(p, pre + ".mlp.linear1.bias", {m}, true, false, false);
  b.fc2_w = add_param(p, pre + ".mlp.linear2.weight", {d, m}, true, true, true);
  b.fc2_b = add_param(p, pre + ".mlp.linear2.bias", {d}, true, false, false);
  return b;
}

constexpr int kMaxT = 112;
struct TransposeTable {
  int n;
  int tile_start[kMaxT + 1];
  int rows[kMaxT], cols[kMaxT];
  long long src[kMaxT], dst[kMaxT];
};

__global__ void __launch_bounds__(256) transpose_cast_batched_kernel(const float* __restrict__ src, bf16* __restrict__ dst,
                                                                     TransposeTable t) {
  __shared__ float tile[64][65];
  int lo = 0, hi = t.n;
  while (hi - lo > 1) {
    const int mid = (lo + hi) >> 1;
    if (t.tile_start[mid] <= (int)blockIdx.x) lo = mid; else hi = mid;
  }
  const int rows = t.rows[lo], cols = t.cols[lo];
  const int local = blockIdx.x - t.tile_start[lo];
  const int tcols = (cols + 63) >> 6;
  const int r0 = (local / tcols) * 64, c0 = (local % tcols) * 64;
  const float* s = src + t.src[lo];
  bf16* d = dst + t.dst[lo];
  const int q = threadIdx.x & 15, rr = threadIdx.x >> 4;
  const bool vec = (cols & 3) == 0 && (rows & 3) == 0;
  if (vec) {
#pragma unroll
    for (int i = 0; i < 4; ++i) {
      const int r = r0 + rr + 16 * i, c = c0 + q * 4;
      f32x4 v = {0, 0, 0, 0};
      if (r < rows && c < cols) v = Vec4<float>::load(s + (size_t)r * cols + c);
#pragma unroll
      for (int e = 0; e < 4; ++e) tile[rr + 16 * i][q * 4 + e] = v[e];
    }
    __syncthreads();
#pragma unroll
    for (int i = 0; i < 4; ++i) {
      const int c = c0 + rr + 16 * i, r = r0 + q * 4;
      if (c < cols && r < rows) {
        const f32x4 v = {tile[q * 4 + 0][rr + 16 * i], tile[q * 4 + 1][rr + 16 * i], tile[q * 4 + 2][rr + 16 * i], tile[q * 4 + 3][rr + 16 * i]};
        Vec4<bf16>::store(d + (size_t)c * rows + r, v);
      }
    }
    return;
  }
  const int tx = threadIdx.x & 63, ty = threadIdx.x >> 6;
  for (int i = ty; i < 64; i += 4) {
    const int r = r0 + i, c = c0 + tx;
    tile[i][tx] = (r < rows && c < cols) ? s[(size_t)r * cols + c] : 0.f;
  }
  __syncthreads();
  for (int i = ty; i < 64; i += 4) {
    const int c = c0 + i, r = r0 + tx;
    if (c < cols && r < rows) d[(size_t)c * rows + r] = (bf16)tile[tx][i];
  }
}

struct WsAlloc {
  size_t cur = 0;
  size_t take(size_t bytes) {
    size_t o = cur;
    cur += align_up(bytes ? bytes : 16, 256);
    return o;
  }
};

BlockA alloc_block(WsAlloc& w, size_t M, size_t d, size_t m, size_t heads_tokens, size_t es) {
  BlockA a;
  a.x1 = w.take(M * d * es);
  a.mean1 = w.take(M * 4);
  a.rstd1 = w.take(M * 4);
  a.qkv = w.take(M * 3 * d * es);
  a.o = w.take(M * d * es);
  a.lse = w.take(heads_tokens * 4);
  a.h_mid = w.take(M * d * 4);
  a.x2 = w.take(M * d * es);
  a.mean2 = w.take(M * 4);
  a.rstd2 = w.take(M * 4);
  a.u = w.take(M * m * es);
  a.g = w.take(M * m * es);
  return a;
}

#define RC(x)            \
  do {                   \
    int _rc = (x);       \
    if (_rc) return _rc; \
  } while (0)

constexpr float kRmsEps = 1e-6f;

int norm_fwd(hct_mae_plan* p, const float* x, const float* gamma, const float* beta, int rows, int D, float eps, void* y, int y_dtype,
             float* mean, float* rstd, hipStream_t s) {
  if (p->norm_kind == 1) return hct_rmsnorm_fwd(x, gamma, rows, D, kRmsEps, y, y_dtype, rstd, s);
  return hct_layernorm_fwd(x, gamma, beta, rows, D, eps, y, y_dtype, mean, rstd, s);
}

int norm_bwd(hct_mae_plan* p, const void* dy, int dy_dtype, const float* x, const float* mean, const float* rstd, const float* gamma,
             const float* dres, const int32_t* dres_rows, int rows, int D, float* dx, void* dx_shadow, int shadow_dtype, float* dgamma,
             float* dbeta, float* dcolsum, void* workspace, size_t workspace_bytes, hipStream_t s) {
  if (p->norm_kind == 1)
    return hct_rmsnorm_bwd_mapped(dy, dy_dtype, x, rstd, gamma, dres, dres_rows, rows, D, dx, dx_shadow, shadow_dtype, dgamma, dcolsum,
                                  workspace, workspace_bytes, s);
  return hct_layernorm_bwd_mapped(dy, dy_dtype, x, mean, rstd, gamma, dres, dres_rows, rows, D, dx, dx_shadow, shadow_dtype, dgamma, dbeta,
                                  dcolsum, workspace, workspace_bytes, s);
}

int norm_bwd_plain(hct_mae_plan* p, const void* dy, int dy_dtype, const float* x, const float* mean, const float* rstd, const float* gamma,
                   const float* dres, int rows, int D, float* dx, void* dx_shadow, int shadow_dtype, float* dgamma, float* dbeta,
                   float* dcolsum, void* workspace, size_t workspace_bytes, hipStream_t s) {
  return norm_bwd(p, dy, dy_dtype, x, mean, rstd, gamma, dres, nullptr, rows, D, dx, dx_shadow, shadow_dtype, dgamma, dbeta, dcolsum, workspace,
                  workspace_bytes, s);
}

hct_gemm_args base_args() {
  hct_gemm_args a;
  memset(&a, 0, sizeof(a));
  a.alpha = 1.0f;
  return a;
}

int nt_gemm(hct_mae_plan* p, hct_gemm_args& a, hipStream_t s) {
  if (p->s_nt_bytes == 0) return hct_gemm(&a, a.colsum_out ? p->ws + p->s_small : nullptr, a.colsum_out ? p->s_small_bytes : 0, s);
  if (!p->nt_ws_armed) {
    if (hipMemsetAsync(p->ws + p->s_small + p->s_small_bytes, 0, p->s_nt_bytes, s) != hipSuccess) {
      set_error("plan: clearing the stream-K region of the GEMM workspace failed");
      return HCT_E_WORKSPACE;
    }
    p->nt_ws_armed = true;
  }
  a.workspace_armed = 1;
  return hct_gemm(&a, p->ws + p->s_small, p->s_small_bytes + p->s_nt_bytes, s);
// ... 507 lines not shown
    const char* ev = getenv("HCT_WGRAD_DEFER");
    p->wg_defer = p->dt == HCT_BF16 && !(ev && ev[0] == '0');
    const char* eb = getenv("HCT_WGRAD_GROUP_BLOCKS");
    p->wg_blocks = eb && *eb ? std::max(0, atoi(eb)) : 0;
    p->s_wg_bytes = hct_gemm_tn_group_workspace_bytes((p->lora > 0 ? 8 : 4) * (c->encoder_depth + p->cfg.decoder_depth) + 4);
    for (int i = 0; i < kWgSlots; ++i) p->s_wg[i] = p->wg_defer ? w.take(p->s_wg_bytes) : 0;
  }
  p->final_off = p->param_elems;
  p->ws_bytes = w.cur;

  auto reg = [&](const std::string& n, size_t off, int64_t r, int64_t cc, int dtp) { p->acts[n] = Act{off, r, cc, dtp}; };
  reg("ids_restore", p->a_ids_restore, batch, p->L, 2);
  reg("ids_shuffle", p->a_ids_shuffle, batch, p->L, 2);
  reg("mask", p->a_mask, batch, p->L, HCT_F32);
  reg("patches", p->a_patches, (int64_t)batch * p->K, p->pd, p->dt);
  reg("tok", p->a_tok, (int64_t)batch * p->K, p->D, p->dt);
  reg("enc_in", p->h_enc[0], p->Me, p->D, HCT_F32);
  for (int i = 0; i < c->encoder_depth; ++i) reg("enc" + std::to_string(i) + ".out", p->h_enc[i + 1], p->Me, p->D, HCT_F32);
  reg("latent", p->a_latent, p->Me, p->D, p->dt);
  reg("dec_in", p->h_dec[0], p->Md, p->Dd, HCT_F32);
  for (int i = 0; i < p->cfg.decoder_depth; ++i) reg("dec" + std::to_string(i) + ".out", p->h_dec[i + 1], p->Md, p->Dd, HCT_F32);
  reg("tail_rows", p->a_tail_rows, 1, p->Mc, 2);
  reg("pred_full", p->a_pred, p->Md, p->pd, p->dt);
  reg("dpred_full", p->a_dpred, p->Md, p->pd, p->dt);
  if (c->encoder_depth > 0) {
    reg("enc0.qkv", p->aenc[0].qkv, p->Me, 3 * p->D, p->dt);
    reg("enc0.attn_o", p->aenc[0].o, p->Me, p->D, p->dt);
    if (p->lora > 0) reg("enc0.lora_t", p->aenc[0].lora_t, p->Me, 2 * p->lora, p->dt);
  }
  return p;
}

void hct_mae_plan_destroy(hct_mae_plan* p) { delete p; }
int hct_mae_plan_num_params(const hct_mae_plan* p) { return (int)p->params.size(); }
int hct_mae_plan_param_info(const hct_mae_plan* p, int index, hct_param_info* out) {
  HCT_REQUIRE(p && out && index >= 0 && index < (int)p->params.size(), "hct_mae_plan_param_info: bad index");
  *out = p->params[index];
  return 0;
}
int64_t hct_mae_plan_param_elems(const hct_mae_plan* p) { return p->param_elems; }
int64_t hct_mae_plan_bf16_t_elems(const hct_mae_plan* p) { return p->bf16t_elems; }
size_t hct_mae_plan_workspace_bytes(const hct_mae_plan* p) { return p->ws_bytes; }
int hct_mae_plan_len_keep(const hct_mae_plan* p) { return p ? p->K : -1; }
int hct_mae_plan_set_requires_grad(hct_mae_plan* p, int index, int flag) {
  HCT_REQUIRE(p && index >= 0 && index < (int)p->params.size(), "hct_mae_plan_set_requires_grad: bad index");
  if (p->params[index].requires_grad != (flag ? 1 : 0)) p->t_all_done = false;
  p->params[index].requires_grad = flag ? 1 : 0;
  return 0;
}
int hct_mae_plan_set_dec0(hct_mae_plan* p, int on) {
  if (!p) return -1;
  p->dec0 = on != 0 && p->dec0_ok;
  return p->dec0 ? 1 : 0;
}
int hct_mae_plan_set_tail(hct_mae_plan* p, int compact) {
  if (!p) return -1;
  p->tail = compact != 0 && p->tail_ok;
  return p->tail ? 1 : 0;
}

int hct_mae_plan_bind(hct_mae_plan* p, float* params, float* grads, void* params_bf16, void* params_bf16_t, void* workspace,
                      size_t workspace_bytes) {
  HCT_REQUIRE(p && params && workspace, "hct_mae_plan_bind: null buffer");
  HCT_REQUIRE(p->dt == HCT_F32 || (params_bf16 && params_bf16_t), "hct_mae_plan_bind: bf16 mode needs the bf16 weight buffers");
  if (workspace_bytes < p->ws_bytes) { set_error("hct_mae_plan_bind: workspace too small"); return HCT_E_WORKSPACE; }
  p->params_f32 = params; p->grads = grads;
  p->params_bf16 = (bf16*)params_bf16; p->params_bf16_t = (bf16*)params_bf16_t;
  p->ws = (unsigned char*)workspace;
  p->nt_ws_armed = false;
  p->t_all_done = false;
  p->fwd_done = false;
  for (auto& v : p->wg_prepared) v.clear();
  p->wg_pending.clear();
  return 0;
}

int hct_mae_refresh_weights(hct_mae_plan* p, int with_plain, void* stream) {
  HCT_REQUIRE(p && p->params_f32, "hct_mae_refresh_weights: plan not bound");
  if (p->dt != HCT_BF16) return 0;
  if (with_plain) RC(hct_cast(p->params_f32, HCT_F32, p->params_bf16, HCT_BF16, p->param_elems, stream));
  TransposeTable t;
  t.n = 0;
  t.tile_start[0] = 0;
  auto flush = [&]() -> int {
    if (t.n == 0) return 0;
    hipLaunchKernelGGL(transpose_cast_batched_kernel, dim3(t.tile_start[t.n]), dim3(256), 0, (hipStream_t)stream, p->params_f32,
                       p->params_bf16_t, t);
    t.n = 0;
    return check_hip(hipGetLastError(), "hct_mae_refresh_weights");
  };
  for (const auto& pi : p->params) {
    if (pi.bf16_t_offset < 0) continue;
    if (!with_plain && p->t_all_done && !pi.requires_grad) continue;
    const int rows = (int)pi.shape[0], cols = (int)(pi.numel / pi.shape[0]);
    t.rows[t.n] = rows; t.cols[t.n] = cols; t.src[t.n] = pi.offset; t.dst[t.n] = pi.bf16_t_offset;
    t.tile_start[t.n + 1] = t.tile_start[t.n] + ((rows + 63) / 64) * ((cols + 63) / 64);
    if (++t.n == kMaxT) RC(flush());
  }
  RC(flush());
  p->t_all_done = true;
  return 0;
}

int hct_mae_forward(hct_mae_plan* p, const void* x, int x_dtype, const float* noise, float* loss, float grad_scale, void* stream) {
  HCT_REQUIRE(p && p->ws && x && noise && loss, "hct_mae_forward: plan not bound or null argument");
  HCT_REQUIRE(!p->vit, "hct_mae_forward: encoder-only plans are driven by hct_vit_forward");
  HCT_REQUIRE(x_dtype == HCT_F32 || x_dtype == HCT_F16, "hct_mae_forward: volumes are fp32 or fp16");
  hipStream_t s = (hipStream_t)stream;
  unsigned char* ws = p->ws;
  const hct_mae_config& c = p->cfg;
  const int B = p->B;
  int32_t* ids_restore = (int32_t*)(ws + p->a_ids_restore);
  int32_t* ids_shuffle = (int32_t*)(ws + p->a_ids_shuffle);
  float* mask = (float*)(ws + p->a_mask);
  RC(hct_mask_rank(noise, B, p->L, p->K, ids_restore, ids_shuffle, mask, s));
  RC(hct_patch_gather(x, x_dtype, ids_shuffle, B, c.in_chans, c.input_size, c.patch_size, p->L, p->K, ws + p->a_patches, p->dt, s));
  RC(linear_fwd(p, ws + p->a_patches, B * p->K, p->pd, p->p_pe_w, p->p_pe_b, p->D, ws + p->a_tok, p->dt, HCT_ACT_NONE, nullptr, nullptr, s));
  RC(hct_encoder_assemble_fwd(ws + p->a_tok, p->dt, p->pf(p->p_cls), p->pf(p->p_pos), ids_shuffle, B, p->L, p->K, p->D, (float*)(ws + p->h_enc[0]), s));
  for (int i = 0; i < c.encoder_depth; ++i)
    RC(block_forward(p, p->enc[i], p->aenc[i], (const float*)(ws + p->h_enc[i]), (float*)(ws + p->h_enc[i + 1]), B, p->Ne, p->D, p->Mlp, p->H, s));
  RC(norm_fwd(p, (const float*)(ws + p->h_enc[c.encoder_depth]), p->pf(p->p_norm_w), p->pf(p->p_norm_b), p->Me, p->D, 1e-5f,
                       ws + p->a_latent, p->dt, (float*)(ws + p->a_lat_mean), (float*)(ws + p->a_lat_rstd), s));
  RC(linear_fwd(p, ws + p->a_latent, p->Me, p->D, p->p_de_w, p->p_de_b, p->Dd, ws + p->a_e, p->dt, HCT_ACT_NONE, nullptr, nullptr, s));
  RC(hct_decoder_assemble_fwd(ws + p->a_e, p->dt, p->pf(p->p_mask), p->pf(p->p_dcls), p->pf(p->p_dpos), ids_restore, B, p->L, p->K, p->Dd,
                              (float*)(ws + p->h_dec[0]), s));
  const bool tail = p->tail && p->tail_ok;
  p->tail_fwd = tail;
  if (tail) RC(hct_tail_rows(ids_restore, B, p->L, p->K, (int32_t*)(ws + p->a_tail_rows), (int32_t*)(ws + p->a_tail_inv), s));
  const bool dec0 = p->dec0 && p->dec0_ok;
  p->dec0_fwd = dec0;
  if (dec0) RC(dec0_index(ids_restore, B, p->L, p->K, (int32_t*)(ws + p->a_kept_rows), (int32_t*)(ws + p->a_cat_idx), s));
  for (int i = 0; i < c.decoder_depth; ++i) {
    if (dec0 && i == 0)
      RC(block_forward_dec0(p, p->dec[i], p->adec[i], (const float*)(ws + p->h_dec[i]), (float*)(ws + p->h_dec[i + 1]), s));
    else if (tail && i == c.decoder_depth - 1)
      RC(block_forward_tail(p, p->dec[i], p->adec[i], (const float*)(ws + p->h_dec[i]), (float*)(ws + p->h_dec[i + 1]), s));
    else
      RC(block_forward(p, p->dec[i], p->adec[i], (const float*)(ws + p->h_dec[i]), (float*)(ws + p->h_dec[i + 1]), B, p->Nd, p->Dd, p->Mlpd, p->Hd, s));
  }
  const int Mt = tail ? p->Mc : p->Md;
  RC(norm_fwd(p, (const float*)(ws + p->h_dec[c.decoder_depth]), p->pf(p->p_dnorm_w), p->pf(p->p_dnorm_b), Mt, p->Dd, 1e-5f,
                       ws + p->a_ynorm, p->dt, (float*)(ws + p->a_yn_mean), (float*)(ws + p->a_yn_rstd), s));
  RC(linear_fwd(p, ws + p->a_ynorm, Mt, p->Dd, p->p_pred_w, p->p_pred_b, p->pd, ws + p->a_pred, p->dt, HCT_ACT_NONE, nullptr, nullptr, s));
  const bool train = grad_scale != 0.0f;
  RC(masked_mse_launch(ws + p->a_pred, p->dt, x, x_dtype, mask, B, c.in_chans, c.input_size, c.patch_size, c.norm_pix_loss,
                       (float)((int64_t)B * (p->L - p->K)), (float*)(ws + p->a_row_loss), loss, train ? ws + p->a_dpred : nullptr, nullptr,
                       train ? grad_scale : 1.0f, s, tail ? ids_shuffle : nullptr, p->K));
  p->fwd_done = true;
  p->dpred_done = train;
  return 0;
}

int hct_vit_forward(hct_mae_plan* p, const void* x, int x_dtype, void* stream) {
  HCT_REQUIRE(x, "hct_vit_forward: null argument");
  return hct_vit_forward_parts(p, &x, 1, x_dtype, stream);
}

int hct_vit_forward_parts(hct_mae_plan* p, const void* const* xs, int n_parts, int x_dtype, void* stream) {
  HCT_REQUIRE(p && p->ws && xs && n_parts > 0, "hct_vit_forward: plan not bound or null argument");
  HCT_REQUIRE(p->vit, "hct_vit_forward: the plan was not created with encoder_only = 1");
  HCT_REQUIRE(x_dtype == HCT_F32 || x_dtype == HCT_F16, "hct_vit_forward: volumes are fp32 or fp16");
  HCT_REQUIRE(p->B % n_parts == 0, "hct_vit_forward_parts: the plan's batch (%d) is not a multiple of the number of parts (%d)", p->B, n_parts);
  hipStream_t s = (hipStream_t)stream;
  unsigned char* ws = p->ws;
  const hct_mae_config& c = p->cfg;
  const int B = p->B, Bp = B / n_parts;
  for (int i = 0; i < n_parts; ++i) {
    HCT_REQUIRE(xs[i], "hct_vit_forward_parts: null part %d", i);
    RC(hct_patch_gather(xs[i], x_dtype, nullptr, Bp, c.in_chans, c.input_size, c.patch_size, p->L, p->L,
                        ws + p->a_patches + (size_t)i * Bp * p->L * p->pd * p->esz(), p->dt, s));
  }
  RC(linear_fwd(p, ws + p->a_patches, B * p->L, p->pd, p->p_pe_w, p->p_pe_b, p->D, ws + p->a_tok, p->dt, HCT_ACT_NONE, nullptr, nullptr, s));
  RC(hct_vit_assemble_fwd(ws + p->a_tok, p->dt, p->pf(p->p_cls), p->p_reg >= 0 ? p->pf(p->p_reg) : nullptr, p->p_pos >= 0 ? p->pf(p->p_pos) : nullptr, B,
                          p->L, p->R, p->D, (float*)(ws + p->h_enc[0]), s));
  for (int i = 0; i < c.encoder_depth; ++i)
    RC(block_forward(p, p->enc[i], p->aenc[i], (const float*)(ws + p->h_enc[i]), (float*)(ws + p->h_enc[i + 1]), B, p->Ne, p->D, p->Mlp, p->H, s));
  RC(norm_fwd(p, (const float*)(ws + p->h_enc[c.encoder_depth]), p->pf(p->p_norm_w), p->pf(p->p_norm_b), p->Me, p->D, p->norm_eps,
                       ws + p->a_latent, p->dt, (float*)(ws + p->a_lat_mean), (float*)(ws + p->a_lat_rstd), s));
  p->fwd_done = true;
  return 0;
}

int hct_vit_backward_stage(hct_mae_plan* p, int stage, const void* dlatent, void* stream) {
  HCT_REQUIRE(p && p->ws && p->grads && p->vit, "hct_vit_backward_stage: plan not bound, no gradient buffer, or not an encoder-only plan");
  if (!p->fwd_done) { set_error("hct_vit_backward_stage: forward has not run"); return HCT_E_STATE; }
  hipStream_t s = (hipStream_t)stream;
  unsigned char* ws = p->ws;
  const int B = p->B, ne = p->cfg.encoder_depth;
  float* dh = (float*)(ws + p->s_dh);
  void* small = ws + p->s_small;
  const int Re = (int)p->genc.size();
  auto enc_out = [&](int i) { return i >= 0 ? p->genc[i % Re].out : p->s_dh_shadow; };
  if (stage == 0) {
    HCT_REQUIRE(dlatent, "hct_vit_backward_stage: stage 0 needs dlatent");
    p->wg_pending.clear(); p->wg_slot = 0; p->wg_blocks_pending = 0; p->final_off = p->param_elems;
    RC(norm_bwd_plain(p, dlatent, p->dt, (const float*)(ws + p->h_enc[ne]), (const float*)(ws + p->a_lat_mean), (const float*)(ws + p->a_lat_rstd),
                         p->pf(p->p_norm_w), nullptr, p->Me, p->D, dh, ws + enc_out(ne - 1), p->dt, p->gf(p->p_norm_w), p->gf(p->p_norm_b),
                         ne > 0 ? p->gf(p->enc[ne - 1].fc2_b) : nullptr, small, p->s_small_bytes, s));
    return end_stage(p, stage, false, false, Re, ne, s);
  }
  if (stage <= ne) {
    const int i = ne - stage;
    RC(block_backward(p, p->enc[i], p->aenc[i], p->genc[i % Re], enc_out(i - 1), (const float*)(ws + p->h_enc[i]), B, p->Ne, p->D, p->Mlp, p->H,
                      i > 0 ? p->enc[i - 1].fc2_b : -1, s));
    return end_stage(p, stage, true, false, Re, ne, s);
  }
  if (stage == ne + 1) {
    void* dtok = ws + p->a_dtok;
    RC(hct_vit_assemble_bwd(dh, B, p->L, p->R, p->D, dtok, p->dt, p->gf(p->tr(p->p_cls)), p->gf(p->tr(p->p_reg)), p->gf(p->tr(p->p_pos)), s));
    RC(linear_wgrad(p, dtok, ws + p->a_patches, B * p->L, p->D, p->pd, p->tr(p->p_pe_w), p->tr(p->p_pe_b), s));
    return end_stage(p, stage, false, false, Re, ne, s);
  }
  set_error("hct_vit_backward_stage: stage %d out of range", stage);
  return HCT_E_BADARG;
}

int hct_mae_set_loss_grad(hct_mae_plan* p, const float* dloss) {
  HCT_REQUIRE(p, "hct_mae_set_loss_grad: null plan");
  p->dloss = dloss;
  return 0;
}

int hct_mae_num_backward_stages(const hct_mae_plan* p) { return (int)p->stage_range.size(); }
int64_t hct_mae_backward_final_offset(const hct_mae_plan* p) { return p ? p->final_off : -1; }
int hct_mae_plan_set_wgrad_defer(hct_mae_plan* p, int defer, int group_blocks) {
  if (!p) return -1;
  p->wg_defer = defer != 0 && p->dt == HCT_BF16 && p->s_wg_bytes > 0 && p->s_wg[kWgSlots - 1] != 0;
  p->wg_blocks = group_blocks > 0 ? group_blocks : 0;
  return p->wg_defer ? 1 : 0;
}
// ... 91 lines not shown
```

### include/headct_hip.h

```cpp
#ifndef HEADCT_HIP_H
#define HEADCT_HIP_H

#include <stddef.h>
#include <stdint.h>

#ifdef __cplusplus
extern "C" {
#endif

#define HCT_F32 0
#define HCT_BF16 1
#define HCT_F16 2

#define HCT_E_BADARG (-1)
#define HCT_E_UNSUPPORTED (-2)
#define HCT_E_WORKSPACE (-3)
#define HCT_E_STATE (-4)

#define HCT_ACT_NONE 0
#define HCT_ACT_GELU 1
#define HCT_ACT_DGELU 2
#define HCT_ACT_TANH 3
#define HCT_ACT_GELU_D 4
#define HCT_ACT_MULAUX 5
// ... 191 lines not shown
                  size_t workspace_bytes, void* params_bf16, void* stream);

typedef struct hct_mae_config {
  int input_size, patch_size, in_chans;
  double mask_ratio;
  int pos_embed;
  int encoder_depth, encoder_embed_dim, encoder_mlp_dim, encoder_num_heads;
  int decoder_depth, decoder_embed_dim, decoder_mlp_dim, decoder_num_heads;
  int norm_pix_loss, use_bias;
  int encoder_only, num_register_tokens;
  float final_norm_eps;
  int lora_rank;
  int norm_kind;
} hct_mae_config;

typedef struct hct_mae_plan hct_mae_plan;

typedef struct hct_param_info {
  char name[96];
  int ndim;
  int64_t shape[5];
  int64_t offset;
  int64_t numel;
  int requires_grad;
  int is_matrix;
  int64_t bf16_t_offset;
} hct_param_info;

hct_mae_plan* hct_mae_plan_create(const hct_mae_config* cfg, int batch, int compute_dtype);
void hct_mae_plan_destroy(hct_mae_plan*);
int hct_mae_plan_num_params(const hct_mae_plan*);
int hct_mae_plan_param_info(const hct_mae_plan*, int index, hct_param_info* out);
int64_t hct_mae_plan_param_elems(const hct_mae_plan*);
int64_t hct_mae_plan_bf16_t_elems(const hct_mae_plan*);
size_t hct_mae_plan_workspace_bytes(const hct_mae_plan*);
int hct_mae_plan_len_keep(const hct_mae_plan*);
int hct_mae_plan_set_tail(hct_mae_plan*, int compact);
int hct_mae_plan_set_dec0(hct_mae_plan*, int on);
int hct_mae_plan_bind(hct_mae_plan*, float* params, float* grads, void* params_bf16, void* params_bf16_t,
                      void* workspace, size_t workspace_bytes);
int hct_mae_refresh_weights(hct_mae_plan*, int with_plain, void* stream);
int hct_mae_forward(hct_mae_plan*, const void* x, int x_dtype, const float* noise, float* loss, float grad_scale, void* stream);
int hct_mae_set_loss_grad(hct_mae_plan*, const float* dloss);
int hct_mae_num_backward_stages(const hct_mae_plan*);
int hct_mae_backward_stage_range(const hct_mae_plan*, int stage, int64_t* begin, int64_t* end);
int hct_mae_backward_stage(hct_mae_plan*, int stage, void* stream);
int64_t hct_mae_backward_final_offset(const hct_mae_plan*);
int hct_mae_plan_set_wgrad_defer(hct_mae_plan*, int defer, int group_blocks);
int hct_mae_plan_set_requires_grad(hct_mae_plan*, int index, int flag);
int hct_vit_forward(hct_mae_plan*, const void* x, int x_dtype, void* stream);
int hct_vit_forward_parts(hct_mae_plan*, const void* const* xs, int n_parts, int x_dtype, void* stream);
int hct_vit_backward_stage(hct_mae_plan*, int stage, const void* dlatent, void* stream);
int hct_vit_assemble_bwd(const float* dh0, int B, int L, int R, int D, void* dtok, int dtok_dtype, float* dcls, float* dreg, float* dpos,
                         void* stream);
int hct_lora_qv_fwd(const void* x1, const void* Aq, const void* Av, const void* Bq, const void* Bv, int B, int N, int H, int dh, int r, int dtype,
                    void* T, void* qkv, void* stream);
size_t hct_lora_qv_bwd_workspace_bytes(int M, int D, int r, int dtype);
int hct_lora_qv_bwd(const void* dqkv, const void* x1, const void* T, const void* Aq, const void* Av, const void* Bq, const void* Bv,
                    const void* AqT, const void* AvT, const void* BqT, const void* BvT, int B, int N, int H, int dh, int r, int dtype, float* dAq,
                    float* dAv, float* dBq, float* dBv, void* dx1, void* workspace, size_t workspace_bytes, void* stream);
int hct_topk_dot_chunks(int Q, int64_t G);
size_t hct_topk_dot_workspace(int Q, int64_t G, int k);
int hct_topk_dot(const void* q, int Q, const void* g, int64_t G, int D, int dtype, const int32_t* exclude, int k, float* scores, int32_t* idx,
                 void* workspace, size_t workspace_bytes, void* stream);
int hct_attention_row_probs(const void* qkv, int B, int N, int H, int dh, int dtype, const int32_t* rows, int n_rows, float* probs, void* stream);
int hct_mae_recon_accum(const void* pred, int pred_dtype, int has_cls_row, const void* x, int x_dtype , const float* mask,
                        int B, int C, int S, int P, int norm_pix, float* recon_sum, float* err_sum, int32_t* cnt, void* stream);
int hct_mae_recon_finish(const float* recon_sum, const float* err_sum, const int32_t* cnt, const void* x, int x_dtype, int B, int C, int S, int P,
                         float* recon, float* err, float* err_vol, void* stream);
const void* hct_mae_plan_activation(const hct_mae_plan*, const char* name, int64_t* rows, int64_t* cols, int* dtype);

void hct_prof_enable(int mask);
void hct_prof_reset(void);
int hct_prof_read(int id, double* total_ms, int64_t* launches, double* work);
int hct_prof_read_bytes(int id, double* bytes);
typedef struct hct_prof_shape {
  int M, N, K, mode, tiles, sk_tiles;
  int64_t launches;
  double total_ms, work, bytes;
} hct_prof_shape;
int hct_prof_shapes(int id, hct_prof_shape* out, int cap);
void hct_debug_force_simple_attention(int mode);
void hct_debug_set_gemm_variant(int v);

#ifdef __cplusplus
}
#endif
#endif
```

Baseline: 7054 CT-volumes/s.

## Add stream-variant knobs: occupancy-sized norm grid and bf16-source weight transpose

Adds a g_stream_variant bitmask that gates several memory-bound kernel variants. The default enables two of them: layernorm/rmsnorm forward grids sized from hipOccupancy resident blocks times CUs instead of a fixed cap of 2048, and the weight-transpose refresh reading from bf16 params instead of fp32 to halve read traffic. Also adds optional variants that are off by default: a paired masked-MSE kernel that handles two adjacent patches per block, a wider unroll plus column-major grid for the decoder reductions, and row prefetch in layernorm. The bf16-sourced transpose relies on params_bf16 being up to date, so it can be wrong if that copy is stale.

```diff
diff --git a/headct_foundation_amd/_lib.py b/headct_foundation_amd/_lib.py
--- a/headct_foundation_amd/_lib.py
+++ b/headct_foundation_amd/_lib.py
@@ -164,6 +164,9 @@
     "hct_lamb_workspace_bytes": (c_size_t, [c_int64, c_int]),
     "hct_lamb_step": (c_int, [c_void_p] * 7 + [c_int, c_int64] + [C.c_double] * 5 + [c_void_p] * 4 + [c_size_t, c_void_p, c_void_p]),
     "hct_debug_set_gemm_variant": (None, [c_int]),
+    "hct_debug_set_stream_variant": (None, [c_int]),
+    "hct_debug_norm_fwd_resident_grid": (c_int, [c_int, c_int, c_int]),
+    "hct_debug_dec0_aggregate": (c_int, [c_void_p, c_int, c_void_p, c_void_p, c_int, c_int, c_int, c_int, c_void_p, c_void_p]),
     "hct_gemm_nt_stream_k_bytes": (c_size_t, []),
     "hct_gemm_tn_group_workspace_bytes": (c_size_t, [c_int]),
     "hct_gemm_tn_group_prepare": (c_int, [c_void_p, c_int, c_void_p, c_size_t, c_void_p]),
diff --git a/headct_foundation_amd/csrc/common.h b/headct_foundation_amd/csrc/common.h
--- a/headct_foundation_amd/csrc/common.h
+++ b/headct_foundation_amd/csrc/common.h
@@ -37,7 +37,8 @@
 
 int masked_mse_launch(const void* pred, int pred_dtype, const void* x, int x_dtype, const float* mask, int B, int C, int S, int P,
                       int norm_pix, float mask_sum, float* row_loss, float* loss, void* dpred, const float* dpred_scale,
-                      float host_scale, hipStream_t s, const int32_t* masked_ids = nullptr, int K = 0);
+                      float host_scale, hipStream_t s, const int32_t* masked_ids = nullptr, int K = 0,
+                      const int32_t* ids_restore = nullptr);
 int dec0_index(const int32_t* ids_restore, int B, int L, int K, int32_t* kept_rows, int32_t* cat_idx, hipStream_t s);
 int dec0_table(const float* mask_token, const float* pos, int L, int D, float* out, hipStream_t s);
 int dec0_aggregate(const void* g, int dtype, const int32_t* kept_rows, const int32_t* ids_restore, int B, int L, int K, int W, void* out, hipStream_t s);
@@ -63,6 +64,27 @@
 extern thread_local FoldSink* g_fold_sink;
 int fold_partials(const FoldJob& job, hipStream_t s);
 int fold_flush(FoldSink& sink, hipStream_t s);
+
+int cus_available();
+int occupancy_blocks_per_cu(const void* kernel, int block, size_t lds);
+template <auto Kernel, int Block>
+inline int resident_blocks_per_cu() {
+  static const int per_cu = occupancy_blocks_per_cu(reinterpret_cast<const void*>(Kernel), Block, 0);
+  return per_cu;
+}
+template <auto Kernel, int Block>
+inline int resident_grid() {
+  return resident_blocks_per_cu<Kernel, Block>() * cus_available();
+}
+
+enum StreamVariant : int {
+  kSvNormGrid = 1,
+  kSvTransBf16 = 2,
+  kSvMsePair = 4,
+  kSvReduce = 8,
+  kSvNormPrefetch = 16,
+};
+extern int g_stream_variant;
 
 inline size_t dtype_size(int dt) { return dt == HCT_BF16 ? 2 : 4; }
 inline size_t align_up(size_t v, size_t a) { return (v + a - 1) / a * a; }
diff --git a/headct_foundation_amd/csrc/elementwise.hip b/headct_foundation_amd/csrc/elementwise.hip
--- a/headct_foundation_amd/csrc/elementwise.hip
+++ b/headct_foundation_amd/csrc/elementwise.hip
@@ -6,6 +6,8 @@
 namespace hct {
 
 static thread_local char g_err[512] = "";
+constexpr int kSvDefault = kSvNormGrid | kSvTransBf16;
+int g_stream_variant = kSvDefault;
 void set_error(const char* fmt, ...) {
   va_list ap;
   va_start(ap, fmt);
@@ -119,21 +121,22 @@
   for (int d = threadIdx.x * 4; d < D; d += blockDim.x * 4) Vec4<T>::store(out + d, Vec4<float>::load(src + d));
 }
 
-__global__ void encoder_assemble_bwd_pos_kernel(const float* __restrict__ dh0, const int32_t* __restrict__ ids_restore,
+template <int U>
+__global__ void __launch_bounds__(256) encoder_assemble_bwd_pos_kernel(const float* __restrict__ dh0, const int32_t* __restrict__ ids_restore,
                                                 int B, int L, int K, int D, float* __restrict__ dpos) {
   const int l = blockIdx.x;
   for (int d = threadIdx.x * 4; d < D; d += blockDim.x * 4) {
     f32x4 acc = {0, 0, 0, 0};
-    for (int b0 = 0; b0 < B; b0 += 8) {
-      int r[8];
-      f32x4 v[8];
-#pragma unroll
-      for (int u = 0; u < 8; ++u) r[u] = b0 + u < B ? ids_restore[(size_t)(b0 + u) * L + l] : K;
-#pragma unroll
-      for (int u = 0; u < 8; ++u)
+    for (int b0 = 0; b0 < B; b0 += U) {
+      int r[U];
+      f32x4 v[U];
+#pragma unroll
+      for (int u = 0; u < U; ++u) r[u] = b0 + u < B ? ids_restore[(size_t)(b0 + u) * L + l] : K;
+#pragma unroll
+      for (int u = 0; u < U; ++u)
         v[u] = r[u] < K ? Vec4<float>::load(dh0 + ((size_t)(b0 + u) * (K + 1) + 1 + r[u]) * D + d) : f32x4{0, 0, 0, 0};
 #pragma unroll
-      for (int u = 0; u < 8; ++u)
+      for (int u = 0; u < U; ++u)
         if (r[u] < K) acc += v[u];
     }
     Vec4<float>::store(dpos + (size_t)l * D + d, acc);
@@ -197,7 +200,7 @@
   }
 }
 
-template <typename T, int NV>
+template <typename T, int NV, bool PF>
 __global__ void __launch_bounds__(256) layernorm_fwd_reg_kernel(const float* __restrict__ x, const float* __restrict__ gamma,
                                                                 const float* __restrict__ beta, int rows, int D, float eps,
                                                                 T* __restrict__ y, float* __restrict__ mean,
@@ -211,16 +214,34 @@
     g[i] = d < D ? Vec4<float>::load(gamma + d) : f32x4{0, 0, 0, 0};
     bt[i] = d < D ? Vec4<float>::load(beta + d) : f32x4{0, 0, 0, 0};
   }
-  for (int row = wid; row < rows; row += nw) {
+  auto load_row = [&](int row, f32x4* v) {
     const float* xr = x + (size_t)row * D;
-    f32x4 v[NV];
-    float s = 0.f;
 #pragma unroll
     for (int i = 0; i < NV; ++i) {
       const int d = lane * 4 + 256 * i;
-      if (d < D) {
-        v[i] = Vec4<float>::load_nt(xr + d);
-        s += (v[i][0] + v[i][1]) + (v[i][2] + v[i][3]);
+      v[i] = d < D ? Vec4<float>::load_nt(xr + d) : f32x4{0, 0, 0, 0};
+    }
+  };
+  f32x4 v[NV], vn[NV];
+  if (PF && wid < rows) load_row(wid, v);
+  for (int row = wid; row < rows; row += nw) {
+    float s = 0.f;
+    if constexpr (PF) {
+      if (row + nw < rows) load_row(row + nw, vn);
+#pragma unroll
+      for (int i = 0; i < NV; ++i) {
+        const int d = lane * 4 + 256 * i;
+        if (d < D) s += (v[i][0] + v[i][1]) + (v[i][2] + v[i][3]);
+      }
+    } else {
+      const float* xr = x + (size_t)row * D;
+#pragma unroll
+      for (int i = 0; i < NV; ++i) {
+        const int d = lane * 4 + 256 * i;
+        if (d < D) {
+          v[i] = Vec4<float>::load_nt(xr + d);
+          s += (v[i][0] + v[i][1]) + (v[i][2] + v[i][3]);
+        }
       }
     }
     const float mu = wave_sum(s) / (float)D;
@@ -247,6 +268,10 @@
         o = o * g[i] + bt[i];
         Vec4<T>::store(yr + d, o);
       }
+    }
+    if (PF) {
+#pragma unroll
+      for (int i = 0; i < NV; ++i) v[i] = vn[i];
     }
   }
 }
@@ -513,22 +538,23 @@
 }
 
 constexpr int kAsmBlocks = 256;
-__global__ void decoder_assemble_bwd_reduce_kernel(const float* __restrict__ dy, const int32_t* __restrict__ ids_shuffle,
+template <int U>
+__global__ void __launch_bounds__(256) decoder_assemble_bwd_reduce_kernel(const float* __restrict__ dy, const int32_t* __restrict__ ids_shuffle,
                                                    int B, int L, int K, int D, float* __restrict__ partial) {
   for (int d = threadIdx.x * 4; d < D; d += blockDim.x * 4) {
     f32x4 am = {0, 0, 0, 0}, ac = {0, 0, 0, 0};
     for (int b = blockIdx.x; b < B; b += gridDim.x) {
       const float* base = dy + (size_t)b * (L + 1) * D;
       ac += Vec4<float>::load(base + d);
-      for (int j0 = K; j0 < L; j0 += 8) {
-        int l[8];
-        f32x4 v[8];
-#pragma unroll
-        for (int u = 0; u < 8; ++u) l[u] = j0 + u < L ? ids_shuffle[(size_t)b * L + j0 + u] : 0;
-#pragma unroll
-        for (int u = 0; u < 8; ++u) v[u] = Vec4<float>::load(base + (size_t)(1 + l[u]) * D + d);
-#pragma unroll
-        for (int u = 0; u < 8; ++u)
+      for (int j0 = K; j0 < L; j0 += U) {
+        int l[U];
+        f32x4 v[U];
+#pragma unroll
+        for (int u = 0; u < U; ++u) l[u] = j0 + u < L ? ids_shuffle[(size_t)b * L + j0 + u] : 0;
+#pragma unroll
+        for (int u = 0; u < U; ++u) v[u] = Vec4<float>::load(base + (size_t)(1 + l[u]) * D + d);
+#pragma unroll
+        for (int u = 0; u < U; ++u)
           if (j0 + u < L) am += v[u];
       }
     }
@@ -631,6 +657,103 @@
   if (threadIdx.x == 0 && row_loss) row_loss[lrow] = sse / (float)pd;
 }
 
+template <typename TX, typename T>
+__global__ void __launch_bounds__(256) masked_mse_pair_kernel(const T* __restrict__ pred, const TX* __restrict__ x,
+                                                              const float* __restrict__ mask, int S, int P, int L, int norm_pix,
+                                                              float inv_masksum, float* __restrict__ row_loss, T* __restrict__ dpred,
+                                                              const float* __restrict__ dscale, float hscale,
+                                                              const int32_t* __restrict__ ids_restore, int K) {
+  __shared__ float s_tmp[4];
+  const int pd = P * P * P;
+  const int g = S / P, gp = (g + 1) >> 1;
+  const int per_vol = g * g * gp;
+  const int b = blockIdx.x / per_vol, rem = blockIdx.x - b * per_vol;
+  const int line = rem / gp, j = rem - line * gp;
+  const int gh = line / g, gw = line - gh * g;
+  const int np = 2 * j + 1 < g ? 2 : 1;
+  bool on[2] = {false, false};
+  const T* prow[2] = {nullptr, nullptr};
+  T* drow[2] = {nullptr, nullptr};
+  size_t lrow[2] = {0, 0};
+  for (int q = 0; q < np; ++q) {
+    const int l = line * g + 2 * j + q;
+    if (ids_restore) {
+      const int rk = ids_restore[(size_t)b * L + l];
+      if (rk < K) continue;
+      lrow[q] = (size_t)b * (L - K) + (rk - K);
+      prow[q] = pred + lrow[q] * pd;
+      if (dpred) drow[q] = dpred + lrow[q] * pd;
+      on[q] = true;
+    } else {
+      const size_t r = (size_t)b * (L + 1) + 1 + l;
+      lrow[q] = (size_t)b * L + l;
+      prow[q] = pred + r * pd;
+      if (dpred) drow[q] = dpred + r * pd;
+      on[q] = mask[lrow[q]] != 0.f;
+      if (!on[q]) {
+        if (threadIdx.x == 0 && row_loss) row_loss[lrow[q]] = 0.f;
+        if (drow[q])
+          for (int k = threadIdx.x * 4; k < pd; k += 1024) Vec4<T>::store(drow[q] + k, f32x4{0, 0, 0, 0});
+      }
+    }
+  }
+  if (!ids_restore && rem == 0 && dpred) {
+    T* crow = dpred + (size_t)b * (L + 1) * pd;
+    for (int k = threadIdx.x * 4; k < pd; k += 1024) Vec4<T>::store(crow + k, f32x4{0, 0, 0, 0});
+  }
+  if (!on[0] && !on[1]) return;
+  const TX* vol = x + (size_t)b * S * S * S + ((size_t)(gh * P) * S + gw * P) * S + (size_t)(2 * j) * P;
+  auto tgt_at = [&](int q, int k) -> float {
+    int u = k;
+    const int pz = u % P; u /= P;
+    const int pw = u % P; u /= P;
+    return to_f32(vol[((size_t)u * S + pw) * S + q * P + pz]);
+  };
+  float mu[2] = {0.f, 0.f}, rsd[2] = {1.f, 1.f};
+  if (norm_pix) {
+    float s[2] = {0.f, 0.f};
+    for (int k = threadIdx.x; k < pd; k += 256)
+      for (int q = 0; q < 2; ++q)
+        if (on[q]) s[q] += tgt_at(q, k);
+    for (int q = 0; q < 2; ++q)
+      if (on[q]) mu[q] = block_sum_256(s[q], s_tmp) / (float)pd;
+    float v[2] = {0.f, 0.f};
+    for (int k = threadIdx.x; k < pd; k += 256)
+      for (int q = 0; q < 2; ++q)
+        if (on[q]) {
+          const float dlt = tgt_at(q, k) - mu[q];
+          v[q] += dlt * dlt;
+        }
+    for (int q = 0; q < 2; ++q)
+      if (on[q]) rsd[q] = 1.0f / sqrtf(block_sum_256(v[q], s_tmp) / (float)(pd - 1) + 1.0e-6f);
+  }
+  const float gscale = 2.0f * inv_masksum / (float)pd * (dscale ? *dscale : 1.0f) * hscale;
+  float sse[2] = {0.f, 0.f};
+  for (int k = threadIdx.x * 4; k < pd; k += 1024) {
+    int u = k;
+    const int pz = u % P; u /= P;
+    const int pw = u % P; u /= P;
+    const TX* tp = vol + ((size_t)u * S + pw) * S + pz;
+    f32x4 tv[2];
+#pragma unroll
+    for (int q = 0; q < 2; ++q)
+      if (on[q]) tv[q] = Vec4<TX>::load(tp + q * P);
+#pragma unroll
+    for (int q = 0; q < 2; ++q)
+      if (on[q]) {
+        const f32x4 t = (tv[q] - mu[q]) * rsd[q];
+        const f32x4 df = Vec4<T>::load(prow[q] + k) - t;
+        sse[q] += (df[0] * df[0] + df[1] * df[1]) + (df[2] * df[2] + df[3] * df[3]);
+        if (drow[q]) Vec4<T>::store(drow[q] + k, df * gscale);
+      }
+  }
+  for (int q = 0; q < 2; ++q)
+    if (on[q]) {
+      const float t = block_sum_256(sse[q], s_tmp);
+      if (threadIdx.x == 0 && row_loss) row_loss[lrow[q]] = t / (float)pd;
+    }
+}
+
 __global__ void __launch_bounds__(256) loss_fold_kernel(const float* __restrict__ row_loss, int n, float inv_masksum,
                                                         float* __restrict__ loss) {
   __shared__ float s_tmp[4];
@@ -1053,10 +1176,10 @@
 
 template <typename T>
 __global__ void __launch_bounds__(256) dec0_table_sum_kernel(const T* __restrict__ g, const int32_t* __restrict__ ids_restore, int B, int L, int K,
-                                                             int W, T* __restrict__ out) {
+                                                             int W, T* __restrict__ out, int by_col) {
   __shared__ f32x4 s_part[4][64];
-  const int l = blockIdx.x, q = threadIdx.x & 63, vg = threadIdx.x >> 6;
-  const int col = blockIdx.y * 256 + q * 4;
+  const int l = by_col ? blockIdx.y : blockIdx.x, q = threadIdx.x & 63, vg = threadIdx.x >> 6;
+  const int col = (by_col ? blockIdx.x : blockIdx.y) * 256 + q * 4;
   f32x4 acc = {0, 0, 0, 0};
   if (col < W) {
     for (int b0 = vg; b0 < B; b0 += 32) {
@@ -1110,6 +1233,12 @@
   }
 }
 
+static void launch_asm_reduce(int nblk, int threads, hipStream_t s, const float* dy, const int32_t* ids_shuffle, int B, int L, int K, int D,
+                              float* partial) {
+  if (g_stream_variant & kSvReduce) hipLaunchKernelGGL(decoder_assemble_bwd_reduce_kernel<32>, dim3(nblk), dim3(threads), 0, s, dy, ids_shuffle, B, L, K, D, partial);
+  else hipLaunchKernelGGL(decoder_assemble_bwd_reduce_kernel<8>, dim3(nblk), dim3(threads), 0, s, dy, ids_shuffle, B, L, K, D, partial);
+}
+
 int scale_unless_one(void* buf, int dtype, int64_t n, const float* scale, hipStream_t s) {
   HCT_REQUIRE(n % 4 == 0 && scale, "scale_unless_one: n %% 4 != 0 or null scale");
   const int blocks = (int)std::min<int64_t>(2048, (n / 4 + 255) / 256);
@@ -1121,7 +1250,7 @@
 
 int masked_mse_launch(const void* pred, int pred_dtype, const void* x, int x_dtype, const float* mask, int B, int C, int S, int P,
                       int norm_pix, float mask_sum, float* row_loss, float* loss, void* dpred, const float* dpred_scale,
-                      float host_scale, hipStream_t s, const int32_t* masked_ids, int K) {
+                      float host_scale, hipStream_t s, const int32_t* masked_ids, int K, const int32_t* ids_restore) {
   HCT_REQUIRE(P % 4 == 0 && S % P == 0 && mask_sum > 0.f, "hct_masked_mse: bad geometry S=%d P=%d mask_sum=%f", S, P, mask_sum);
   HCT_REQUIRE(x_dtype == HCT_F32 || x_dtype == HCT_F16, "hct_masked_mse: volumes are fp32 or fp16");
   const int g = S / P, L = g * g * g;
@@ -1129,6 +1258,20 @@
   HCT_REQUIRE(pd % 4 == 0, "hct_masked_mse: patch dim %% 4 != 0");
   const float inv = 1.0f / mask_sum;
   HCT_REQUIRE(!masked_ids || (K >= 0 && K < L), "hct_masked_mse: compact form needs 0 <= K < L");
+  if ((g_stream_variant & kSvMsePair) && C == 1 && g > 1 && (!masked_ids || ids_restore)) {
+    const int nblk = B * g * g * ((g + 1) / 2);
+    const int32_t* restore = masked_ids ? ids_restore : nullptr;
+#define HCT_MSE_PAIR(TX_)                                                                                                          \
+  HCT_DISPATCH_DTYPE(pred_dtype, T,                                                                                                \
+                     hipLaunchKernelGGL((masked_mse_pair_kernel<TX_, T>), dim3(nblk), dim3(256), 0, s, (const T*)pred, (const TX_*)x, mask, \
+                                        S, P, L, norm_pix, inv, loss ? row_loss : nullptr, (T*)dpred, dpred_scale, host_scale, restore, K))
+    if (x_dtype == HCT_F16) HCT_MSE_PAIR(f16);
+    else HCT_MSE_PAIR(float);
+#undef HCT_MSE_PAIR
+    if (loss) hipLaunchKernelGGL(loss_fold_kernel, dim3(1), dim3(256), 0, s, row_loss, masked_ids ? B * (L - K) : B * L, inv, loss);
+    HCT_CHECK_LAUNCH("hct_masked_mse");
+    return 0;
+  }
   const int nrows = masked_ids ? B * (L - K) : B * (L + 1);
   if (x_dtype == HCT_F16) {
     HCT_DISPATCH_DTYPE(pred_dtype, T,
@@ -1158,8 +1301,9 @@
   HCT_REQUIRE(W % 4 == 0 && (W * dtype_size(dtype)) % 16 == 0, "dec0_aggregate: row width must be a multiple of 16 bytes");
   const int Nc = B * (K + 1);
   if (int rc = hct_gather_rows(g, kept_rows, Nc, (int)(W * dtype_size(dtype)), out, s)) return rc;
-  const dim3 grid(L, (W + 255) / 256);
-  HCT_DISPATCH_DTYPE(dtype, T, hipLaunchKernelGGL(dec0_table_sum_kernel<T>, grid, dim3(256), 0, s, (const T*)g, ids_restore, B, L, K, W, (T*)out + (size_t)Nc * W));
+  const int by_col = (g_stream_variant & kSvReduce) ? 1 : 0;
+  const dim3 grid = by_col ? dim3((W + 255) / 256, L) : dim3(L, (W + 255) / 256);
+  HCT_DISPATCH_DTYPE(dtype, T, hipLaunchKernelGGL(dec0_table_sum_kernel<T>, grid, dim3(256), 0, s, (const T*)g, ids_restore, B, L, K, W, (T*)out + (size_t)Nc * W, by_col));
   HCT_CHECK_LAUNCH("dec0_aggregate");
   return 0;
 }
@@ -1172,7 +1316,7 @@
   const int threads = D / 4 >= 256 ? 256 : (D / 4 > 64 ? 128 : 64);
   const int nblk = std::min(B, kAsmBlocks);
   float* partial = (float*)workspace;
-  hipLaunchKernelGGL(decoder_assemble_bwd_reduce_kernel, dim3(nblk), dim3(threads), 0, s, dh, ids_shuffle, B, L, K, D, partial);
+  launch_asm_reduce(nblk, threads, s, dh, ids_shuffle, B, L, K, D, partial);
   hipLaunchKernelGGL(dec0_token_grads_kernel, dim3((D + 31) / 32), dim3(512), 0, s, partial, nblk, dcat, B, L, K, D, dmask, dcls);
   HCT_CHECK_LAUNCH("dec0_token_grads");
   return 0;
@@ -1183,6 +1327,27 @@
 
 const char* hct_last_error_string(void) { return g_err; }
 int hct_version(void) { return 100; }
+void hct_debug_set_stream_variant(int mask) { g_stream_variant = mask < 0 ? kSvDefault : mask; }
+int hct_debug_dec0_aggregate(const void* g, int dtype, const int32_t* kept_rows, const int32_t* ids_restore, int B, int L, int K, int W, void* out,
+                             void* stream) {
+  HCT_REQUIRE(g && kept_rows && ids_restore && out && B > 0 && L > 0 && K >= 0 && K <= L, "hct_debug_dec0_aggregate: bad arguments");
+  return dec0_aggregate(g, dtype, kept_rows, ids_restore, B, L, K, W, out, (hipStream_t)stream);
+}
+int hct_debug_norm_fwd_resident_grid(int rms, int D, int y_dtype) {
+#define HCT_RG(NV_, ...) (y_dtype == HCT_BF16 ? resident_grid<&__VA_ARGS__<bf16, NV_ HCT_RG_X>, 256>() : resident_grid<&__VA_ARGS__<float, NV_ HCT_RG_X>, 256>())
+#define HCT_RG_D(K_) (D <= 256 ? HCT_RG(1, K_) : D <= 512 ? HCT_RG(2, K_) : D <= 768 ? HCT_RG(3, K_) : D <= 1024 ? HCT_RG(4, K_) : 0)
+#define HCT_RG_X
+  if (rms) return HCT_RG_D(rmsnorm_fwd_reg_kernel);
+#undef HCT_RG_X
+#define HCT_RG_X , true
+  if (g_stream_variant & kSvNormPrefetch) return HCT_RG_D(layernorm_fwd_reg_kernel);
+#undef HCT_RG_X
+#define HCT_RG_X , false
+  return HCT_RG_D(layernorm_fwd_reg_kernel);
+#undef HCT_RG_X
+#undef HCT_RG_D
+#undef HCT_RG
+}
 int hct_has_mfma_kernels(void) { return 1; }
 
 int hct_mask_rank(const float* noise, int B, int L, int K, int32_t* ids_restore, int32_t* ids_shuffle, float* mask,
@@ -1251,7 +1416,10 @@
                        hipLaunchKernelGGL(encoder_assemble_bwd_tok_kernel<T>, dim3(B * K), dim3(threads), 0, s, dh0, K, D,
                                           (T*)dtok));
   if (dcls) hipLaunchKernelGGL(strided_rowsum_kernel, dim3((D + 255) / 256), dim3(256), 0, s, dh0, B, (size_t)(K + 1) * D, D, dcls);
-  if (dpos) hipLaunchKernelGGL(encoder_assemble_bwd_pos_kernel, dim3(L), dim3(threads), 0, s, dh0, ids_restore, B, L, K, D, dpos);
+  if (dpos) {
+    if (g_stream_variant & kSvReduce) hipLaunchKernelGGL(encoder_assemble_bwd_pos_kernel<32>, dim3(L), dim3(threads), 0, s, dh0, ids_restore, B, L, K, D, dpos);
+    else hipLaunchKernelGGL(encoder_assemble_bwd_pos_kernel<8>, dim3(L), dim3(threads), 0, s, dh0, ids_restore, B, L, K, D, dpos);
+  }
   HCT_CHECK_LAUNCH("hct_encoder_assemble_bwd");
   return 0;
 }
@@ -1272,15 +1440,25 @@
   return 0;
 }
 
+static int norm_fwd_grid(int rows, int resident) {
+  const int cap = (g_stream_variant & kSvNormGrid) && resident > 0 ? resident : 2048;
+  return min((rows + 3) / 4, cap);
+}
+
 int hct_layernorm_fwd(const float* x, const float* gamma, const float* beta, int rows, int D, float eps, void* y,
                       int y_dtype, float* mean, float* rstd, void* stream) {
   HCT_REQUIRE(D % 4 == 0 && rows >= 0, "hct_layernorm_fwd: bad shape rows=%d D=%d", rows, D);
   if (rows == 0) return 0;
-  const int nblk = min((rows + 3) / 4, 2048);
-#define HCT_LN_FWD(NV_)                                                                                                 \
+#define HCT_LN_FWD_PF(NV_, PF_)                                                                                         \
   HCT_DISPATCH_DTYPE(y_dtype, T,                                                                                       \
-                     hipLaunchKernelGGL((layernorm_fwd_reg_kernel<T, NV_>), dim3(nblk), dim3(256), 0, (hipStream_t)stream, x, \
-                                        gamma, beta, rows, D, eps, (T*)y, mean, rstd))
+                     hipLaunchKernelGGL((layernorm_fwd_reg_kernel<T, NV_, PF_>),                                        \
+                                        dim3(norm_fwd_grid(rows, resident_grid<&layernorm_fwd_reg_kernel<T, NV_, PF_>, 256>())), dim3(256), 0, \
+                                        (hipStream_t)stream, x, gamma, beta, rows, D, eps, (T*)y, mean, rstd))
+#define HCT_LN_FWD(NV_)                                          \
+  do {                                                           \
+    if (g_stream_variant & kSvNormPrefetch) HCT_LN_FWD_PF(NV_, true); \
+    else HCT_LN_FWD_PF(NV_, false);                              \
+  } while (0)
   if (D <= 256) HCT_LN_FWD(1);
   else if (D <= 512) HCT_LN_FWD(2);
   else if (D <= 768) HCT_LN_FWD(3);
@@ -1290,6 +1468,7 @@
                        hipLaunchKernelGGL(layernorm_fwd_kernel<T>, dim3((rows + 3) / 4), dim3(256), 0, (hipStream_t)stream,
                                           x, gamma, beta, rows, D, eps, (T*)y, mean, rstd));
 #undef HCT_LN_FWD
+#undef HCT_LN_FWD_PF
   HCT_CHECK_LAUNCH("hct_layernorm_fwd");
   return 0;
 }
@@ -1337,11 +1516,11 @@
                     void* stream) {
   HCT_REQUIRE(D % 4 == 0 && rows >= 0, "hct_rmsnorm_fwd: bad shape rows=%d D=%d", rows, D);
   if (rows == 0) return 0;
-  const int nblk = min((rows + 3) / 4, 2048);
-#define HCT_RMS_FWD(NV_)                                                                                                     \
+#define HCT_RMS_FWD(NV_)                                                                      \
   HCT_DISPATCH_DTYPE(y_dtype, T,                                                                                             \
-                     hipLaunchKernelGGL((rmsnorm_fwd_reg_kernel<T, NV_>), dim3(nblk), dim3(256), 0, (hipStream_t)stream, x, gamma, \
-                                        rows, D, eps, (T*)y, rstd))
+                     hipLaunchKernelGGL((rmsnorm_fwd_reg_kernel<T, NV_>),                                                     \
+                                        dim3(norm_fwd_grid(rows, resident_grid<&rmsnorm_fwd_reg_kernel<T, NV_>, 256>())), dim3(256), 0, \
+                                        (hipStream_t)stream, x, gamma, rows, D, eps, (T*)y, rstd))
   if (D <= 256) HCT_RMS_FWD(1);
   else if (D <= 512) HCT_RMS_FWD(2);
   else if (D <= 768) HCT_RMS_FWD(3);
@@ -1419,7 +1598,7 @@
                                         ids_shuffle, L, K, D, (T*)de));
   const int nblk = min(B, kAsmBlocks);
   float* partial = (float*)workspace;
-  hipLaunchKernelGGL(decoder_assemble_bwd_reduce_kernel, dim3(nblk), dim3(threads), 0, s, dy, ids_shuffle, B, L, K, D, partial);
+  launch_asm_reduce(nblk, threads, s, dy, ids_shuffle, B, L, K, D, partial);
   hipLaunchKernelGGL(fold_partials_kernel, dim3((D + 31) / 32, 2), dim3(kFoldThreads), 0, s, partial, nblk, 2, D, dmask_token,
                      ddec_cls, (float*)nullptr);
   HCT_CHECK_LAUNCH("hct_decoder_assemble_bwd");
diff --git a/headct_foundation_amd/csrc/gemm.hip b/headct_foundation_amd/csrc/gemm.hip
--- a/headct_foundation_amd/csrc/gemm.hip
+++ b/headct_foundation_amd/csrc/gemm.hip
@@ -1636,6 +1636,16 @@
 
 static int num_cus() { return std::max(8, num_cus_total() - g_cu_reserve); }
 
+int cus_available() { return num_cus(); }
+int occupancy_blocks_per_cu(const void* kernel, int block, size_t lds) {
+  int n = 0;
+  if (hipOccupancyMaxActiveBlocksPerMultiprocessor(&n, kernel, block, lds) != hipSuccess) {
+    (void)hipGetLastError();
+    return 0;
+  }
+  return n;
+}
+
 static bool aligned_to(const void* p, size_t a) { return p == nullptr || ((uintptr_t)p % a) == 0; }
 
 static Epilogue make_epilogue(const hct_gemm_args* a) {
diff --git a/headct_foundation_amd/csrc/mae_plan.hip b/headct_foundation_amd/csrc/mae_plan.hip
--- a/headct_foundation_amd/csrc/mae_plan.hip
+++ b/headct_foundation_amd/csrc/mae_plan.hip
@@ -145,7 +145,8 @@
   long long src[kMaxT], dst[kMaxT];
 };
 
-__global__ void __launch_bounds__(256) transpose_cast_batched_kernel(const float* __restrict__ src, bf16* __restrict__ dst,
+template <typename TI>
+__global__ void __launch_bounds__(256) transpose_cast_batched_kernel(const TI* __restrict__ src, bf16* __restrict__ dst,
                                                                      TransposeTable t) {
   __shared__ float tile[64][65];
   int lo = 0, hi = t.n;
@@ -157,7 +158,7 @@
   const int local = blockIdx.x - t.tile_start[lo];
   const int tcols = (cols + 63) >> 6;
   const int r0 = (local / tcols) * 64, c0 = (local % tcols) * 64;
-  const float* s = src + t.src[lo];
+  const TI* s = src + t.src[lo];
   bf16* d = dst + t.dst[lo];
   const int q = threadIdx.x & 15, rr = threadIdx.x >> 4;
   const bool vec = (cols & 3) == 0 && (rows & 3) == 0;
@@ -166,7 +167,7 @@
     for (int i = 0; i < 4; ++i) {
       const int r = r0 + rr + 16 * i, c = c0 + q * 4;
       f32x4 v = {0, 0, 0, 0};
-      if (r < rows && c < cols) v = Vec4<float>::load(s + (size_t)r * cols + c);
+      if (r < rows && c < cols) v = Vec4<TI>::load(s + (size_t)r * cols + c);
 #pragma unroll
       for (int e = 0; e < 4; ++e) tile[rr + 16 * i][q * 4 + e] = v[e];
     }
@@ -184,7 +185,7 @@
   const int tx = threadIdx.x & 63, ty = threadIdx.x >> 6;
   for (int i = ty; i < 64; i += 4) {
     const int r = r0 + i, c = c0 + tx;
-    tile[i][tx] = (r < rows && c < cols) ? s[(size_t)r * cols + c] : 0.f;
+    tile[i][tx] = (r < rows && c < cols) ? to_f32(s[(size_t)r * cols + c]) : 0.f;
   }
   __syncthreads();
   for (int i = ty; i < 64; i += 4) {
@@ -858,10 +859,15 @@
   TransposeTable t;
   t.n = 0;
   t.tile_start[0] = 0;
+  const bool from_bf16 = (g_stream_variant & kSvTransBf16) && !with_plain && p->t_all_done && p->params_bf16;
   auto flush = [&]() -> int {
     if (t.n == 0) return 0;
-    hipLaunchKernelGGL(transpose_cast_batched_kernel, dim3(t.tile_start[t.n]), dim3(256), 0, (hipStream_t)stream, p->params_f32,
-                       p->params_bf16_t, t);
+    if (from_bf16)
+      hipLaunchKernelGGL(transpose_cast_batched_kernel<bf16>, dim3(t.tile_start[t.n]), dim3(256), 0, (hipStream_t)stream,
+                         (const bf16*)p->params_bf16, p->params_bf16_t, t);
+    else
+      hipLaunchKernelGGL(transpose_cast_batched_kernel<float>, dim3(t.tile_start[t.n]), dim3(256), 0, (hipStream_t)stream,
+                         (const float*)p->params_f32, p->params_bf16_t, t);
     t.n = 0;
     return check_hip(hipGetLastError(), "hct_mae_refresh_weights");
   };
@@ -921,7 +927,7 @@
   const bool train = grad_scale != 0.0f;
   RC(masked_mse_launch(ws + p->a_pred, p->dt, x, x_dtype, mask, B, c.in_chans, c.input_size, c.patch_size, c.norm_pix_loss,
                        (float)((int64_t)B * (p->L - p->K)), (float*)(ws + p->a_row_loss), loss, train ? ws + p->a_dpred : nullptr, nullptr,
-                       train ? grad_scale : 1.0f, s, tail ? ids_shuffle : nullptr, p->K));
+                       train ? grad_scale : 1.0f, s, tail ? ids_shuffle : nullptr, p->K, ids_restore));
   p->fwd_done = true;
   p->dpred_done = train;
   return 0;
diff --git a/include/headct_hip.h b/include/headct_hip.h
--- a/include/headct_hip.h
+++ b/include/headct_hip.h
@@ -297,6 +297,10 @@
 int hct_prof_shapes(int id, hct_prof_shape* out, int cap);
 void hct_debug_force_simple_attention(int mode);
 void hct_debug_set_gemm_variant(int v);
+void hct_debug_set_stream_variant(int mask);
+int hct_debug_norm_fwd_resident_grid(int rms, int D, int y_dtype);
+int hct_debug_dec0_aggregate(const void* g, int dtype, const int32_t* kept_rows, const int32_t* ids_restore, int B, int L, int K, int W,
+                             void* out, void* stream);
 
 #ifdef __cplusplus
 }
```

After: 7063 CT-volumes/s, median of 6. About the same (+0.1%).
